# JacksonCampolattaro/spectrogram-rs

Hardware: AMD Instinct MI355X
Metric: STFT frames/sec (4096-pt, hop 256) (higher is better)
Workload: dtype f32

## Files before the change

bindings/rust/sgx_sys.rs:

```rust
use std::os::raw::{c_char, c_int, c_void};

#[repr(C)]
pub struct SgxConfig {
    pub struct_size: u32,
    pub sample_rate: f32, pub period: f32, pub stride: f32,
    pub window_samples: u32, pub hop_samples: u32, pub channels: u32, pub rows: u32,
    pub f_min: f64, pub f_max: f64,
    pub min_db: f32, pub max_db: f32,
    pub interp: u32, pub lut_index_mode: u32,
    pub device: i32, pub flags: u32,
}
#[repr(C)] pub struct SgxCtx { _private: [u8; 0] }
#[repr(C)] pub struct SgxFbank { _private: [u8; 0] }

extern "C" {
    pub fn sgx_config_init(cfg: *mut SgxConfig) -> c_int;
    pub fn sgx_create(cfg: *const SgxConfig, out: *mut *mut SgxCtx) -> c_int;
    pub fn sgx_destroy(ctx: *mut SgxCtx);
    pub fn sgx_last_error(ctx: *const SgxCtx) -> *const c_char;
    pub fn sgx_num_frames(ctx: *const SgxCtx, n_samples: usize) -> usize;
    pub fn sgx_process_one(ctx: *mut SgxCtx, h_lr: *const f32, n_avail: usize, h_out: *mut f32) -> c_int;
    pub fn sgx_stft_batch(ctx: *mut SgxCtx, d_pcm: *const f32, n_samples: usize, first_frame: usize,
                          max_frames: usize, d_mags: *mut f32, n_out: *mut usize) -> c_int;
    pub fn sgx_stft_batch_f16(ctx: *mut SgxCtx, d_pcm: *const f32, n_samples: usize, first_frame: usize,
                              max_frames: usize, d_mags_f16: *mut c_void, n_out: *mut usize) -> c_int;
    pub fn sgx_stft_batch_complex(ctx: *mut SgxCtx, d_pcm: *const f32, n_samples: usize, first_frame: usize,
                                  max_frames: usize, d_spec: *mut f32, n_out: *mut usize) -> c_int;
    pub fn sgx_istft_batch(ctx: *mut SgxCtx, d_spec: *const f32, n_frames: usize, first_sample: usize,
                           max_samples: usize, d_pcm: *mut f32, n_out: *mut usize) -> c_int;
    pub fn sgx_istft_supported(ctx: *const SgxCtx) -> c_int;
    pub fn sgx_render_batch(ctx: *mut SgxCtx, d_pcm: *const f32, n_samples: usize, first_frame: usize,
                            max_frames: usize, d_rgba: *mut u8, n_out: *mut usize) -> c_int;
    pub fn sgx_magnitude_in(ctx: *mut SgxCtx, d_mags: *const f32, n_columns: usize, h_ranges: *const f32,
                            n_ranges: u32, d_out: *mut f32) -> c_int;
    pub fn sgx_bands_batch(ctx: *mut SgxCtx, d_pcm: *const f32, n_samples: usize, first_frame: usize,
                           max_frames: usize, d_bands: *mut f32, n_out: *mut usize) -> c_int;
    pub fn sgx_bands_fused(ctx: *const SgxCtx) -> c_int;
    pub fn sgx_bands_peak_batch(ctx: *mut SgxCtx, d_pcm: *const f32, n_samples: usize, first_frame: usize, max_frames: usize,
                                group: usize, d_peak: *mut f32, n_out: *mut usize) -> c_int;
    pub fn sgx_bands_peak_fused(ctx: *const SgxCtx) -> c_int;
    pub fn sgx_psd_batch(ctx: *mut SgxCtx, d_pcm: *const f32, n_samples: usize, first_frame: usize, max_frames: usize,
                         group: usize, d_psd: *mut f32, n_out: *mut usize) -> c_int;
    pub fn sgx_csd_batch(ctx: *mut SgxCtx, d_pcm: *const f32, n_samples: usize, first_frame: usize, max_frames: usize,
                         group: usize, d_csd: *mut f32, n_out: *mut usize) -> c_int;
    pub fn sgx_psd_mags(ctx: *mut SgxCtx, d_mags: *const f32, n_frames: usize, group: usize, d_psd: *mut f32,
                        n_out: *mut usize) -> c_int;
    pub fn sgx_csd_spec(ctx: *mut SgxCtx, d_spec: *const f32, n_frames: usize, group: usize, d_csd: *mut f32,
                        n_out: *mut usize) -> c_int;
    pub fn sgx_psd_fused(ctx: *const SgxCtx) -> c_int;
    pub fn sgx_csd_fused(ctx: *const SgxCtx) -> c_int;
    pub fn sgx_render_bands(ctx: *mut SgxCtx, d_bands: *const f32, n_columns: usize, d_rgba: *mut u8) -> c_int;
    pub fn sgx_fbank_create(ctx: *mut SgxCtx, n_filters: u32, h_first: *const u32, h_count: *const u32, h_weights: *const f32,
                            power: u32, out_fbank: *mut *mut SgxFbank) -> c_int;
    pub fn sgx_fbank_destroy(fbank: *mut SgxFbank);
    pub fn sgx_fbank_filters(fbank: *const SgxFbank) -> u32;
    pub fn sgx_fbank_batch(fbank: *mut SgxFbank, d_pcm: *const f32, n_samples: usize, first_frame: usize, max_frames: usize,
                           d_out: *mut f32, n_out: *mut usize) -> c_int;
    pub fn sgx_fbank_mags(fbank: *mut SgxFbank, d_mags: *const f32, n_columns: usize, d_out: *mut f32) -> c_int;
    pub fn sgx_fbank_fused(fbank: *const SgxFbank) -> c_int;
    pub fn sgx_fbank_cross_batch(fbank: *mut SgxFbank, d_pcm: *const f32, n_samples: usize, first_frame: usize, max_frames: usize,
                                 d_out: *mut f32, n_out: *mut usize) -> c_int;
    pub fn sgx_fbank_cross_spec(fbank: *mut SgxFbank, d_spec: *const f32, n_columns: usize, d_out: *mut f32) -> c_int;
    pub fn sgx_fbank_cross_fused(fbank: *const SgxFbank) -> c_int;
    pub fn sgx_mel_weights(sample_rate: f64, window_samples: u32, n_mels: u32, f_min: f64, f_max: f64, scale: u32, norm: u32,
                           h_first: *mut u32, h_count: *mut u32, h_weights: *mut f32, n_weights: *mut usize) -> c_int;
    pub fn sgx_set_gradient(ctx: *mut SgxCtx, h_rgb: *const u8, n: u32, stereo: c_int) -> c_int;
    pub fn sgx_set_gradient_fn(ctx: *mut SgxCtx, eval: extern "C" fn(f64, *mut u8, *mut c_void), user: *mut c_void,
                               stereo: c_int) -> c_int;
    pub fn sgx_set_builtin_scheme(ctx: *mut SgxCtx, name: *const c_char, stereo: c_int) -> c_int;
    pub fn sgx_lookup_table(ctx: *mut SgxCtx, resolution: u32, h_out: *mut f32) -> c_int;
    pub fn sgx_sync(ctx: *mut SgxCtx) -> c_int;
    pub fn sgx_set_cu_limit(ctx: *mut SgxCtx, n: u32) -> c_int;
    pub fn sgx_cu_limit(ctx: *const SgxCtx) -> u32;
}
extern "C" {
    pub fn hipMalloc(p: *mut *mut c_void, bytes: usize) -> c_int;
    pub fn hipFree(p: *mut c_void) -> c_int;
    pub fn hipMemcpy(dst: *mut c_void, src: *const c_void, bytes: usize, kind: c_int) -> c_int;
}
pub const HIP_MEMCPY_HOST_TO_DEVICE: c_int = 1;
pub const HIP_MEMCPY_DEVICE_TO_HOST: c_int = 2;
pub const SGX_FLAG_PAIRED_FRAMES: u32 = 1024;
pub const SGX_FLAG_COMPLEX_MONO: u32 = 512;
pub const SGX_FLAG_LARGE_TRANSFORM: u32 = 4096;
pub const SGX_MEL_HTK: u32 = 0;
pub const SGX_MEL_SLANEY: u32 = 1;
pub const SGX_MEL_NORM_NONE: u32 = 0;
pub const SGX_MEL_NORM_SLANEY: u32 = 1;
pub const SGX_LIVE_BANDS: c_int = 3;
```

include/sgx.h:

```cpp
#ifndef SGX_H
#define SGX_H

#include <stddef.h>
#include <stdint.h>

#ifdef __cplusplus
extern "C" {
#endif

#if defined(__GNUC__)
#define SGX_API __attribute__((visibility("default")))
#else
#define SGX_API
#endif

typedef enum sgx_status {
    SGX_OK = 0,
    SGX_ERR_INVALID_ARG = -1,
    SGX_ERR_UNSUPPORTED = -2,
    SGX_ERR_HIP = -3,
    SGX_ERR_NOMEM = -4,
    SGX_ERR_NO_DEVICE = -5
} sgx_status;

#define SGX_INTERP_CUBIC 0u
#define SGX_INTERP_COSINE 1u

#define SGX_LUT_FLOOR_N 0u
#define SGX_LUT_ROUND_NM1 1u

typedef struct sgx_ctx sgx_ctx;

typedef struct sgx_config {
    uint32_t struct_size;
    float sample_rate;
    float period;
    float stride;
    uint32_t window_samples;
    uint32_t hop_samples;
    uint32_t channels;
    uint32_t rows;
    double f_min, f_max;
    float min_db, max_db;
    uint32_t interp;
    uint32_t lut_index_mode;
    int32_t device;
    uint32_t flags;
} sgx_config;

#define SGX_FLAG_FORCE_GENERIC 1u
#define SGX_FLAG_NO_FUSED_RENDER 4u
#define SGX_FLAG_PAIRED_FRAMES 1024u
#define SGX_FLAG_COMPLEX_MONO 512u
#define SGX_FLAG_LUT_WALK 64u
#define SGX_FLAG_MIXED_GENERIC 256u
#define SGX_FLAG_LARGE_TRANSFORM 4096u

typedef struct sgx_info {
    uint32_t struct_size;
    uint32_t window_samples;
    uint32_t fft_length;
    uint32_t num_frequencies;
    uint32_t hop_samples;
    uint32_t channels;
    uint32_t pairs;
    uint32_t rows;
    uint32_t sample_rate_u32;
    uint32_t total_samples_per_column;
    uint32_t stft_kernel;
    uint32_t render_path;
    uint64_t mags_bytes_per_frame;
    uint64_t rgba_bytes_per_frame;
} sgx_info;


SGX_API const char *sgx_version(void);

SGX_API int sgx_config_init(sgx_config *cfg);

SGX_API int sgx_create(const sgx_config *cfg, sgx_ctx **out_ctx);
SGX_API void sgx_destroy(sgx_ctx *ctx);

SGX_API const char *sgx_last_error(const sgx_ctx *ctx);

SGX_API int sgx_query(const sgx_ctx *ctx, sgx_info *out);

SGX_API size_t sgx_num_frames(const sgx_ctx *ctx, size_t n_samples);

SGX_API int sgx_set_stream(sgx_ctx *ctx, void *stream);
SGX_API int sgx_sync(sgx_ctx *ctx);

SGX_API int sgx_set_cu_limit(sgx_ctx *ctx, uint32_t n);
SGX_API uint32_t sgx_cu_limit(const sgx_ctx *ctx);


SGX_API int sgx_stft_batch(sgx_ctx *ctx, const float *d_pcm, size_t n_samples, size_t first_frame,
                           size_t max_frames, float *d_mags, size_t *n_out);

SGX_API int sgx_stft_batch_complex(sgx_ctx *ctx, const float *d_pcm, size_t n_samples, size_t first_frame,
                                   size_t max_frames, float *d_spec, size_t *n_out);

SGX_API int sgx_istft_batch(sgx_ctx *ctx, const float *d_spec, size_t n_frames, size_t first_sample,
                            size_t max_samples, float *d_pcm, size_t *n_out);
SGX_API int sgx_istft_supported(const sgx_ctx *ctx);

SGX_API int sgx_stft_batch_f16(sgx_ctx *ctx, const float *d_pcm, size_t n_samples, size_t first_frame,
                               size_t max_frames, void *d_mags_f16, size_t *n_out);

SGX_API int sgx_process_one(sgx_ctx *ctx, const float *h_lr, size_t n_avail, float *h_out);


SGX_API int sgx_render_batch(sgx_ctx *ctx, const float *d_pcm, size_t n_samples, size_t first_frame,
                             size_t max_frames, uint8_t *d_rgba, size_t *n_out);

SGX_API int sgx_render_mags(sgx_ctx *ctx, const float *d_mags, size_t n_columns, uint8_t *d_rgba);

SGX_API int sgx_magnitude_in(sgx_ctx *ctx, const float *d_mags, size_t n_columns, const float *h_ranges,
                             uint32_t n_ranges, float *d_out);

SGX_API int sgx_bands_batch(sgx_ctx *ctx, const float *d_pcm, size_t n_samples, size_t first_frame,
                            size_t max_frames, float *d_bands, size_t *n_out);
SGX_API int sgx_bands_fused(const sgx_ctx *ctx);

SGX_API int sgx_bands_peak_batch(sgx_ctx *ctx, const float *d_pcm, size_t n_samples, size_t first_frame, size_t max_frames,
                                 size_t group, float *d_peak, size_t *n_out);
SGX_API int sgx_bands_peak_fused(const sgx_ctx *ctx);

SGX_API int sgx_psd_batch(sgx_ctx *ctx, const float *d_pcm, size_t n_samples, size_t first_frame, size_t max_frames,
                          size_t group, float *d_psd, size_t *n_out);
SGX_API int sgx_csd_batch(sgx_ctx *ctx, const float *d_pcm, size_t n_samples, size_t first_frame, size_t max_frames,
                          size_t group, float *d_csd, size_t *n_out);
SGX_API int sgx_psd_mags(sgx_ctx *ctx, const float *d_mags, size_t n_frames, size_t group, float *d_psd, size_t *n_out);
SGX_API int sgx_csd_spec(sgx_ctx *ctx, const float *d_spec, size_t n_frames, size_t group, float *d_csd, size_t *n_out);
SGX_API int sgx_psd_fused(const sgx_ctx *ctx);
SGX_API int sgx_csd_fused(const sgx_ctx *ctx);
typedef struct sgx_fbank sgx_fbank;

SGX_API int sgx_fbank_create(sgx_ctx *ctx, uint32_t n_filters, const uint32_t *h_first, const uint32_t *h_count,
                             const float *h_weights, uint32_t power, void **out_fbank);
SGX_API void sgx_fbank_destroy(void *fbank);
SGX_API uint32_t sgx_fbank_filters(const void *fbank);
SGX_API int sgx_fbank_batch(void *fbank, const float *d_pcm, size_t n_samples, size_t first_frame, size_t max_frames,
                            float *d_out, size_t *n_out);
SGX_API int sgx_fbank_mags(void *fbank, const float *d_mags, size_t n_columns, float *d_out);
SGX_API int sgx_fbank_fused(const void *fbank);

SGX_API int sgx_fbank_cross_batch(void *fbank, const float *d_pcm, size_t n_samples, size_t first_frame, size_t max_frames,
                                  float *d_out, size_t *n_out);
SGX_API int sgx_fbank_cross_spec(void *fbank, const float *d_spec, size_t n_columns, float *d_out);
SGX_API int sgx_fbank_cross_fused(const void *fbank);

#define SGX_MEL_HTK 0u
#define SGX_MEL_SLANEY 1u
#define SGX_MEL_NORM_NONE 0u
#define SGX_MEL_NORM_SLANEY 1u
SGX_API int sgx_mel_weights(double sample_rate, uint32_t window_samples, uint32_t n_mels, double f_min, double f_max, uint32_t scale,
                            uint32_t norm, uint32_t *h_first, uint32_t *h_count, float *h_weights, size_t *n_weights);

SGX_API int sgx_render_bands(sgx_ctx *ctx, const float *d_bands, size_t n_columns, uint8_t *d_rgba);

SGX_API int sgx_spectrum_levels(sgx_ctx *ctx, const float *d_column, uint32_t n_bars, double *h_levels);


typedef struct sgx_live sgx_live;

#define SGX_LIVE_MAGS 0
#define SGX_LIVE_MAGS_F16 1
#define SGX_LIVE_RGBA 2
#define SGX_LIVE_BANDS 3

#define SGX_LIVE_REFERENCE_SKIP 1u

SGX_API int sgx_live_create(sgx_ctx *ctx, size_t capacity_pairs, uint32_t flags, sgx_live **out);
SGX_API void sgx_live_destroy(sgx_live *live);
SGX_API long long sgx_live_push(sgx_live *live, const float *h_samples, size_t n_values, uint32_t channels);
SGX_API size_t sgx_live_occupied(const sgx_live *live);
SGX_API int sgx_live_tick(sgx_live *live, int what, void *h_out, size_t max_frames, size_t *n_frames);


SGX_API int sgx_set_gradient(sgx_ctx *ctx, const uint8_t *h_rgb, uint32_t n, int stereo);
typedef void (*sgx_gradient_fn)(double t, uint8_t rgb_out[3], void *user);
SGX_API int sgx_set_gradient_fn(sgx_ctx *ctx, sgx_gradient_fn eval, void *user, int stereo);
SGX_API int sgx_set_builtin_gradient(sgx_ctx *ctx, const char *name);
SGX_API int sgx_set_builtin_scheme(sgx_ctx *ctx, const char *name, int stereo);
SGX_API int sgx_builtin_gradient_eval(const char *name, double t, uint8_t rgb_out[3]);
SGX_API int sgx_builtin_gradient(const char *name, uint8_t *h_rgb_out );

SGX_API int sgx_lookup_table(sgx_ctx *ctx, uint32_t resolution, float *h_out);


SGX_API int sgx_bin_edges(const sgx_ctx *ctx, float *h_out);
SGX_API int sgx_row_sample_counts(const sgx_ctx *ctx, uint32_t *h_out);
SGX_API int sgx_window(const sgx_ctx *ctx, float *h_out);

typedef struct sgx_view sgx_view;
SGX_API int sgx_view_create(sgx_ctx *ctx, uint32_t viewport_frames , sgx_view **out);
SGX_API void sgx_view_destroy(sgx_view *view);
SGX_API int sgx_view_write_rows(sgx_view *view, const void *d_rows_f16, size_t n_rows, uint32_t *offset_out);
SGX_API uint32_t sgx_view_offset(const sgx_view *view);
SGX_API int sgx_live_tick_view(sgx_live *live, sgx_view *view, size_t max_frames, size_t *n_frames);
SGX_API int sgx_view_draw(sgx_view *view, uint32_t width, uint32_t height, float *d_rgba_f32);

typedef struct sgx_image sgx_image;
SGX_API int sgx_image_create(sgx_ctx *ctx, uint32_t width , sgx_image **out);
SGX_API void sgx_image_destroy(sgx_image *image);
SGX_API int sgx_image_write_columns(sgx_image *image, const uint8_t *d_rgba, size_t n_columns, uint32_t *offset_out);
SGX_API uint32_t sgx_image_offset(const sgx_image *image);
SGX_API uint32_t sgx_image_width(const sgx_image *image);
SGX_API uint32_t sgx_image_height(const sgx_image *image);
SGX_API int sgx_live_tick_image(sgx_live *live, sgx_image *image, size_t max_frames, size_t *n_frames);
SGX_API int sgx_image_read(sgx_image *image, int scrolled, uint8_t *d_out);
SGX_API const uint8_t *sgx_image_pixels(const sgx_image *image);


SGX_API int sgx_synth_white_noise(sgx_ctx *ctx, float *d_out, uint64_t first, size_t n_samples,
                                  uint32_t channels, uint32_t seed);
SGX_API int sgx_checksum(sgx_ctx *ctx, const void *d_buf, size_t n_bytes, uint64_t base_word, uint64_t *h_out);
SGX_API int sgx_checksum_add(sgx_ctx *ctx, const void *d_buf, size_t n_bytes, uint64_t base_word, uint64_t *d_acc);

#ifdef __cplusplus
}
#endif
#endif
```

spectrogram_rs_amd/_lib.py:

```python
from __future__ import annotations

import ctypes as C
import os

_HERE = os.path.dirname(os.path.abspath(__file__))
LIB_PATH = os.environ.get("SGX_LIB", os.path.join(_HERE, "libsgx.so"))

SGX_OK = 0
SGX_ERR_INVALID_ARG = -1
SGX_ERR_UNSUPPORTED = -2
SGX_ERR_HIP = -3
SGX_ERR_NOMEM = -4
SGX_ERR_NO_DEVICE = -5

INTERP_CUBIC, INTERP_COSINE = 0, 1
LUT_FLOOR_N, LUT_ROUND_NM1 = 0, 1
FLAG_FORCE_GENERIC = 1
FLAG_NO_FUSED_RENDER = 4
FLAG_LUT_WALK = 64
FLAG_MIXED_GENERIC = 256
FLAG_COMPLEX_MONO = 512
FLAG_PAIRED_FRAMES = 1024
FLAG_LARGE_TRANSFORM = 4096
LIVE_MAGS, LIVE_MAGS_F16, LIVE_RGBA, LIVE_BANDS = 0, 1, 2, 3
LIVE_REFERENCE_SKIP = 1
MEL_HTK, MEL_SLANEY = 0, 1
MEL_NORM_NONE, MEL_NORM_SLANEY = 0, 1


class SgxError(RuntimeError):
    def __init__(self, code: int, message: str):
        super().__init__(f"sgx error {code}: {message}")
        self.code = code


class sgx_config(C.Structure):
    _fields_ = [
        ("struct_size", C.c_uint32),
        ("sample_rate", C.c_float),
        ("period", C.c_float),
        ("stride", C.c_float),
        ("window_samples", C.c_uint32),
        ("hop_samples", C.c_uint32),
        ("channels", C.c_uint32),
        ("rows", C.c_uint32),
        ("f_min", C.c_double),
        ("f_max", C.c_double),
        ("min_db", C.c_float),
        ("max_db", C.c_float),
        ("interp", C.c_uint32),
        ("lut_index_mode", C.c_uint32),
        ("device", C.c_int32),
        ("flags", C.c_uint32),
    ]


class sgx_info(C.Structure):
    _fields_ = [
        ("struct_size", C.c_uint32),
        ("window_samples", C.c_uint32),
        ("fft_length", C.c_uint32),
        ("num_frequencies", C.c_uint32),
        ("hop_samples", C.c_uint32),
        ("channels", C.c_uint32),
        ("pairs", C.c_uint32),
        ("rows", C.c_uint32),
        ("sample_rate_u32", C.c_uint32),
        ("total_samples_per_column", C.c_uint32),
        ("stft_kernel", C.c_uint32),
        ("render_path", C.c_uint32),
        ("mags_bytes_per_frame", C.c_uint64),
        ("rgba_bytes_per_frame", C.c_uint64),
    ]


_vp, _sz = C.c_void_p, C.c_size_t
_ctx = C.c_void_p
SIGNATURES = [
    ("sgx_version", C.c_char_p, []),
    ("sgx_config_init", C.c_int, [C.POINTER(sgx_config)]),
    ("sgx_create", C.c_int, [C.POINTER(sgx_config), C.POINTER(_ctx)]),
    ("sgx_destroy", None, [_ctx]),
    ("sgx_last_error", C.c_char_p, [_ctx]),
    ("sgx_query", C.c_int, [_ctx, C.POINTER(sgx_info)]),
    ("sgx_num_frames", _sz, [_ctx, _sz]),
    ("sgx_set_stream", C.c_int, [_ctx, _vp]),
    ("sgx_sync", C.c_int, [_ctx]),
    ("sgx_set_cu_limit", C.c_int, [_ctx, C.c_uint32]),
    ("sgx_cu_limit", C.c_uint32, [_ctx]),
    ("sgx_stft_batch", C.c_int, [_ctx, _vp, _sz, _sz, _sz, _vp, C.POINTER(_sz)]),
    ("sgx_stft_batch_f16", C.c_int, [_ctx, _vp, _sz, _sz, _sz, _vp, C.POINTER(_sz)]),
    ("sgx_stft_batch_complex", C.c_int, [_ctx, _vp, _sz, _sz, _sz, _vp, C.POINTER(_sz)]),
    ("sgx_istft_batch", C.c_int, [_ctx, _vp, _sz, _sz, _sz, _vp, C.POINTER(_sz)]),
    ("sgx_istft_supported", C.c_int, [_ctx]),
    ("sgx_process_one", C.c_int, [_ctx, _vp, _sz, _vp]),
    ("sgx_render_batch", C.c_int, [_ctx, _vp, _sz, _sz, _sz, _vp, C.POINTER(_sz)]),
    ("sgx_render_mags", C.c_int, [_ctx, _vp, _sz, _vp]),
    ("sgx_magnitude_in", C.c_int, [_ctx, _vp, _sz, _vp, C.c_uint32, _vp]),
    ("sgx_bands_batch", C.c_int, [_ctx, _vp, _sz, _sz, _sz, _vp, C.POINTER(_sz)]),
    ("sgx_bands_fused", C.c_int, [_ctx]),
    ("sgx_bands_peak_batch", C.c_int, [_ctx, _vp, _sz, _sz, _sz, _sz, _vp, C.POINTER(_sz)]),
    ("sgx_bands_peak_fused", C.c_int, [_ctx]),
    ("sgx_psd_batch", C.c_int, [_ctx, _vp, _sz, _sz, _sz, _sz, _vp, C.POINTER(_sz)]),
    ("sgx_csd_batch", C.c_int, [_ctx, _vp, _sz, _sz, _sz, _sz, _vp, C.POINTER(_sz)]),
    ("sgx_psd_mags", C.c_int, [_ctx, _vp, _sz, _sz, _vp, C.POINTER(_sz)]),
    ("sgx_csd_spec", C.c_int, [_ctx, _vp, _sz, _sz, _vp, C.POINTER(_sz)]),
    ("sgx_psd_fused", C.c_int, [_ctx]),
    ("sgx_csd_fused", C.c_int, [_ctx]),
    ("sgx_render_bands", C.c_int, [_ctx, _vp, _sz, _vp]),
    ("sgx_fbank_create", C.c_int, [_ctx, C.c_uint32, _vp, _vp, _vp, C.c_uint32, C.POINTER(_vp)]),
    ("sgx_fbank_destroy", None, [_vp]),
    ("sgx_fbank_filters", C.c_uint32, [_vp]),
    ("sgx_fbank_batch", C.c_int, [_vp, _vp, _sz, _sz, _sz, _vp, C.POINTER(_sz)]),
    ("sgx_fbank_mags", C.c_int, [_vp, _vp, _sz, _vp]),
    ("sgx_fbank_fused", C.c_int, [_vp]),
    ("sgx_fbank_cross_batch", C.c_int, [_vp, _vp, _sz, _sz, _sz, _vp, C.POINTER(_sz)]),
    ("sgx_fbank_cross_spec", C.c_int, [_vp, _vp, _sz, _vp]),
    ("sgx_fbank_cross_fused", C.c_int, [_vp]),
    ("sgx_mel_weights", C.c_int, [C.c_double, C.c_uint32, C.c_uint32, C.c_double, C.c_double, C.c_uint32, C.c_uint32, _vp, _vp, _vp,
                                  C.POINTER(_sz)]),
    ("sgx_spectrum_levels", C.c_int, [_ctx, _vp, C.c_uint32, _vp]),
    ("sgx_live_create", C.c_int, [_ctx, _sz, C.c_uint32, C.POINTER(_vp)]),
    ("sgx_live_destroy", None, [_vp]),
    ("sgx_live_push", C.c_longlong, [_vp, _vp, _sz, C.c_uint32]),
    ("sgx_live_occupied", _sz, [_vp]),
    ("sgx_live_tick", C.c_int, [_vp, C.c_int, _vp, _sz, C.POINTER(_sz)]),
    ("sgx_set_gradient", C.c_int, [_ctx, _vp, C.c_uint32, C.c_int]),
    ("sgx_set_gradient_fn", C.c_int, [_ctx, _vp, _vp, C.c_int]),
    ("sgx_set_builtin_gradient", C.c_int, [_ctx, C.c_char_p]),
    ("sgx_builtin_gradient", C.c_int, [C.c_char_p, _vp]),
    ("sgx_lookup_table", C.c_int, [_ctx, C.c_uint32, _vp]),
    ("sgx_bin_edges", C.c_int, [_ctx, _vp]),
    ("sgx_row_sample_counts", C.c_int, [_ctx, _vp]),
    ("sgx_window", C.c_int, [_ctx, _vp]),
    ("sgx_synth_white_noise", C.c_int, [_ctx, _vp, C.c_uint64, _sz, C.c_uint32, C.c_uint32]),
    ("sgx_set_builtin_scheme", C.c_int, [_ctx, C.c_char_p, C.c_int]),
    ("sgx_builtin_gradient_eval", C.c_int, [C.c_char_p, C.c_double, C.POINTER(C.c_uint8)]),
    ("sgx_view_create", C.c_int, [_ctx, C.c_uint32, C.POINTER(C.c_void_p)]),
    ("sgx_view_destroy", None, [C.c_void_p]),
    ("sgx_view_write_rows", C.c_int, [C.c_void_p, _vp, _sz, C.POINTER(C.c_uint32)]),
    ("sgx_view_offset", C.c_uint32, [C.c_void_p]),
    ("sgx_live_tick_view", C.c_int, [C.c_void_p, C.c_void_p, _sz, C.POINTER(_sz)]),
    ("sgx_view_draw", C.c_int, [C.c_void_p, C.c_uint32, C.c_uint32, _vp]),
    ("sgx_image_create", C.c_int, [_ctx, C.c_uint32, C.POINTER(C.c_void_p)]),
    ("sgx_image_destroy", None, [C.c_void_p]),
    ("sgx_image_write_columns", C.c_int, [C.c_void_p, _vp, _sz, C.POINTER(C.c_uint32)]),
    ("sgx_image_offset", C.c_uint32, [C.c_void_p]),
    ("sgx_image_width", C.c_uint32, [C.c_void_p]),
    ("sgx_image_height", C.c_uint32, [C.c_void_p]),
    ("sgx_live_tick_image", C.c_int, [C.c_void_p, C.c_void_p, _sz, C.POINTER(_sz)]),
    ("sgx_image_read", C.c_int, [C.c_void_p, C.c_int, _vp]),
    ("sgx_image_pixels", C.c_void_p, [C.c_void_p]),
    ("sgx_checksum", C.c_int, [_ctx, _vp, _sz, C.c_uint64, C.POINTER(C.c_uint64)]),
    ("sgx_checksum_add", C.c_int, [_ctx, _vp, _sz, C.c_uint64, _vp]),
]

GRADIENT_FN = C.CFUNCTYPE(None, C.c_double, C.POINTER(C.c_uint8), C.c_void_p)

_lib = None


def load():
    global _lib
    if _lib is not None:
        return _lib
    if not os.path.exists(LIB_PATH):
        raise ImportError(
            f"{LIB_PATH} is missing: build the HIP extension first "
            "(python -c 'import __graft_entry__ as g; g.build()' or make -C spectrogram_rs_amd/csrc). "
            "There is no CPU fallback."
        )
    import torch

    lib = C.CDLL(LIB_PATH, mode=C.RTLD_GLOBAL)
    for name, restype, argtypes in SIGNATURES:
        fn = getattr(lib, name)
        fn.restype = restype
        fn.argtypes = argtypes
    _lib = lib
    return lib
```

spectrogram_rs_amd/csrc/sgx_internal.hpp:

```cpp
#pragma once

#include <hip/hip_runtime.h>

#include <cstdint>
#include <array>
#include <memory>
#include <string>
#include <vector>

#include "../../include/sgx.h"
#include "device_buffer.hpp"
#include "unit_root.hpp"

namespace sgx {

#ifdef __HIPCC__
typedef float sgx_f2v __attribute__((ext_vector_type(2)));
__device__ __forceinline__ float2 cubic_pair(float2 y0, float2 y1, float2 y2, float2 y3, float mu, float mu2, float mu3)
{
    const sgx_f2v Y0 = {y0.x, y0.y}, Y1 = {y1.x, y1.y}, Y2 = {y2.x, y2.y}, Y3 = {y3.x, y3.y};
    const sgx_f2v a0 = ((Y3 - Y2) - Y0) + Y1;
    const sgx_f2v a1 = (Y0 - Y1) - a0;
    const sgx_f2v a2 = Y2 - Y0;
    const sgx_f2v r = ((a0 * mu3) + (a1 * mu2)) + ((a2 * mu) + Y1);
    return make_float2(r.x, r.y);
}
#endif

constexpr int kTCells = 512;
__host__ __device__ inline int sgx_t_cell(double t)
{
    const double x = (t + 1.0) * (double)(kTCells / 2);
    return x >= (double)kTCells ? kTCells - 1 : (x > 0.0 ? (int)x : 0);
}

struct RowEntry {
    uint32_t first;
    uint32_t count;
    float count_f;
    uint32_t pad;
};

struct SampleEntry {
    int32_t i0;
    union { int32_t i1; float w0; };
    float w1;
    float w2;
};
static_assert(sizeof(SampleEntry) == 16, "SampleEntry must be 16 bytes");

struct Tables {
    std::vector<float> window;
    std::vector<float2> twiddle;
    std::vector<float> edges;
    std::vector<RowEntry> rows;
    std::vector<SampleEntry> samples;
};

struct Palette {
    std::vector<uint8_t> rgb;
    uint32_t n = 0;
    int stereo = 0;
    std::vector<float> lut_thr;
    std::vector<float> alpha_thr;
    bool segments = false;
    sgx_gradient_fn fn = nullptr;
    void *fn_user = nullptr;
    std::vector<double> t_thr;
    std::vector<uint16_t> t_cell;
    uint8_t nan_rgb[3] = {0, 0, 0};
};

void build_tables(uint32_t W, uint32_t R, uint32_t sample_rate_u32, double f_min, double f_max, uint32_t interp,
                  Tables &out);
void build_range_tables(uint32_t W, uint32_t sample_rate_u32, uint32_t interp, const float *range_f0, const float *range_f1,
                        uint32_t n_ranges, std::vector<RowEntry> &rows, std::vector<SampleEntry> &samples);
void build_palette_thresholds(float min_db, float max_db, uint32_t lut_mode, Palette &pal);
void build_palette_segments(float min_db, float max_db, Palette &pal);
int lut_index_host(double t, uint32_t n, uint32_t mode);
uint8_t alpha_u8_host(float alpha);
float bounded_db_host(float min_db, float max_db, float power);

enum StftKernel : int { kKernelGeneric = 0, kKernelWg4096 = 2, kKernelChirp = 4, kKernelMixed = 6, kKernelW4800 = 9, kKernelW16384 = 10, kKernelLarge = 11 };

namespace wg { struct WgTables; }
namespace wgr { struct RealTables; }
namespace mix { struct MixTables; struct ChirpTables; }
namespace w48 { struct W48Tables; }
namespace blu { struct BluTables; }
namespace w16k { struct TablesW; }
namespace large { struct LargeTables; }
namespace istft { struct ITables; }
struct TablesDelete {
    void operator()(wg::WgTables *t) const;
    void operator()(wgr::RealTables *t) const;
    void operator()(mix::MixTables *t) const;
    void operator()(mix::ChirpTables *t) const;
    void operator()(w48::W48Tables *t) const;
    void operator()(blu::BluTables *t) const;
    void operator()(w16k::TablesW *t) const;
    void operator()(large::LargeTables *t) const;
    void operator()(istft::ITables *t) const;
};
template <typename T> using TablesPtr = std::unique_ptr<T, TablesDelete>;

inline float2 unit_root2(unsigned long long e, unsigned long long n) { const UnitRoot w = unit_root(e, n); return make_float2(w.re, w.im); }

}

struct sgx_ctx {
    sgx_config cfg{};
    uint32_t W = 0, P = 0, M = 0, H = 0, C = 0, pairs = 0, R = 0, sr_u32 = 0, logP = 0;
    int device = 0;
    hipStream_t stream = nullptr;
    hipEvent_t rebind_event = nullptr;
    sgx::StftKernel stft_kernel = sgx::kKernelGeneric;

    sgx::Tables tab;
    sgx::Palette pal;

    sgx::DeviceBuffer<float> d_window;
    sgx::DeviceBuffer<float2> d_twiddle;
    sgx::DeviceBuffer<sgx::RowEntry> d_rows;
    sgx::DeviceBuffer<sgx::SampleEntry> d_samples;
    sgx::DeviceBuffer<float> d_lut_thr;
    sgx::DeviceBuffer<float> d_alpha_thr;
    sgx::DeviceBuffer<uchar4> d_lut_rgba;
    sgx::DeviceBuffer<uint2> d_pal_seed;
    sgx::DeviceBuffer<double> d_t_thr;
    sgx::DeviceBuffer<uint16_t> d_t_cell;
    sgx::TablesPtr<sgx::wg::WgTables> wg;
    sgx::TablesPtr<sgx::blu::BluTables> blu;
    sgx::TablesPtr<sgx::mix::MixTables> mix;
    sgx::TablesPtr<sgx::w48::W48Tables> w4800;
    sgx::TablesPtr<sgx::wgr::RealTables> real;
    sgx::TablesPtr<sgx::mix::ChirpTables> chz;
    sgx::TablesPtr<sgx::w16k::TablesW> w16k;
    sgx::TablesPtr<sgx::large::LargeTables> large;
    sgx::TablesPtr<sgx::istft::ITables> istft;

    sgx::DeviceBuffer<float> d_ws_mags;
    sgx::DeviceBuffer<float> d_one_in, d_one_out;
    sgx::DeviceBuffer<unsigned long long> d_cksum;
    std::vector<float> bands_key;
    sgx::DeviceBuffer<sgx::RowEntry> d_band_rows;
    sgx::DeviceBuffer<sgx::SampleEntry> d_band_samples;
    sgx::DeviceBuffer<float> d_levels;
    sgx::DeviceBuffer<double> d_psd_carry;

    unsigned long long palette_gen = 0;

    int n_cu = 256;
    int n_cu_device = 256;
    size_t lds_optin = 64 * 1024;
    mutable std::vector<std::pair<std::array<size_t, 3>, int>> occupancy_cache;
    std::vector<struct sgx_view *> views;
    std::vector<struct sgx_image *> images;
    std::vector<struct sgx_fbank *> fbanks;

    std::string err;

    ~sgx_ctx();
};

namespace sgx {

enum class Out { kMags, kMagsF16, kComplex, kRgba, kBands, kPeak, kFbank, kFbankCross, kPsd, kCsd };
struct StftCall {
    const float *pcm;
    uint32_t channels, pairs;
    size_t first, n, total;
    void *out;
    Out kind;
    size_t peak_group;
    const struct sgx_fbank *bank = nullptr;
};
hipError_t launch_generic(const sgx_ctx *c, const StftCall &call);
hipError_t launch_wg4096(const sgx_ctx *c, const StftCall &call);
hipError_t launch_w16384(const sgx_ctx *c, const StftCall &call);
hipError_t launch_w4800(const sgx_ctx *c, const StftCall &call);
hipError_t launch_mixed(const sgx_ctx *c, const StftCall &call);
hipError_t launch_chirpz(const sgx_ctx *c, const StftCall &call);
hipError_t launch_bluestein(const sgx_ctx *c, const StftCall &call);
hipError_t launch_large(const sgx_ctx *c, const StftCall &call);

inline bool paired_mono(const sgx_ctx *c, uint32_t channels)
{
    return channels == 1 && (c->cfg.flags & SGX_FLAG_PAIRED_FRAMES) && !(c->cfg.flags & SGX_FLAG_COMPLEX_MONO);
}
inline bool descriptor_pairs_fit(uint32_t H, uint32_t W) { return 4ull * ((unsigned long long)H + W) <= 0x7fffffffull; }
struct RunSplit { unsigned long long per, blocks; };
inline RunSplit runs_of(unsigned long long n_jobs, unsigned long long per) { return {per, (n_jobs + per - 1) / per}; }
inline RunSplit run_split(const sgx_ctx *c, unsigned long long n_jobs, unsigned per_cu)
{
    const unsigned long long blocks = (unsigned long long)c->n_cu * per_cu, per = (n_jobs + blocks - 1) / blocks;
    return runs_of(n_jobs, per < 1 ? 1 : per);
}
inline bool fast4096_supported(const sgx_ctx *c) { return c->W == 2048; }
hipError_t wg4096_init(sgx_ctx *c);
bool wg4096_can_fuse_render(const sgx_ctx *c);
bool wg4096_can_fuse_bands(const sgx_ctx *c);
bool wg4096_can_fuse_peak(const sgx_ctx *c);
hipError_t launch_deinterleave_pairs(const sgx_ctx *c, const float *d_pcm, float *d_planes, size_t plane_floats, size_t first_sample, size_t n_samples,
                                     uint32_t channels, uint32_t pairs);
bool wg4096_seed_is_within_one(const sgx_ctx *c);
void lut_seed_coefficients(const sgx_ctx *c, float &a, float &b);
namespace wg { bool seed_within_one(const std::vector<float> &thr, double guess_a, double guess_b); }
bool w16384_supported(const sgx_ctx *c);
hipError_t w16384_init(sgx_ctx *c);
hipError_t real4096_init(sgx_ctx *c);
bool real4096_serves(const sgx_ctx *c, const float *d_pcm, uint32_t channels);
bool w4800_supported(const sgx_ctx *c);
hipError_t w4800_init(sgx_ctx *c);
bool mixed_supported(uint32_t W);
hipError_t mixed_init(sgx_ctx *c);
hipError_t mixed_length_tables(uint32_t n, TablesPtr<mix::MixTables> &out);
uint32_t mixed_fixed_plan(const sgx_ctx *c);
bool mixed_real_serves(const sgx_ctx *c, uint32_t channels);
bool chirpz_supported(uint32_t W);
hipError_t chirpz_init(sgx_ctx *c);
bool chirpz_real_serves(const sgx_ctx *c, uint32_t channels);
bool mixed_can_fuse_render(const sgx_ctx *c);
bool mixed_can_fuse_bands(const sgx_ctx *c);
bool bluestein_supported(uint32_t W);
hipError_t bluestein_init(sgx_ctx *c);
bool large_supported(uint32_t W);
hipError_t large_init(sgx_ctx *c);
int istft_route(const sgx_ctx *c);
hipError_t istft_init(sgx_ctx *c);
hipError_t launch_istft(const sgx_ctx *c, const float *d_spec, size_t n_frames, size_t s0, size_t s1, float *d_pcm);
hipError_t launch_to_half(const sgx_ctx *c, const float *d_in, void *d_out, size_t n_pairs);
hipError_t launch_render(const sgx_ctx *c, const float *d_mags, size_t n_columns, uint8_t *d_rgba);
hipError_t launch_magnitude_in(const sgx_ctx *c, const float *d_mags, size_t n_columns, const RowEntry *d_rows,
                               const SampleEntry *d_samples, uint32_t n_ranges, float *d_out);
inline size_t peak_columns(size_t n_src, size_t group, size_t sub)
{
    const size_t spc = (group + sub - 1) / sub, full = n_src / group, rem = n_src - full * group;
    return full * spc + (rem + sub - 1) / sub;
}
hipError_t launch_bands_peak(const sgx_ctx *c, const float *d_src, size_t n_src, size_t group, size_t sub, float *d_dst, bool accumulate);
hipError_t launch_render_bands(const sgx_ctx *c, const float *d_bands, size_t n_columns, uint8_t *d_rgba);
void detach_views(sgx_ctx *c);
void detach_images(sgx_ctx *c);
sgx_ctx *image_context(const struct sgx_image *im);
sgx_ctx *view_context(const struct sgx_view *v);
hipError_t launch_white_noise(const sgx_ctx *c, float *d_out, uint64_t first, size_t n, uint32_t channels, uint32_t seed);
hipError_t launch_checksum(const sgx_ctx *c, const uint32_t *d_words, size_t n_words, uint64_t base_word,
                           unsigned long long *d_acc);

}

#ifdef __HIPCC__
__device__ __forceinline__ void st_stream(float2 *p, float a, float b)
{
    *p = make_float2(a, b);
}

#if SGX_STAMPS
#define SGX_STAMP(i) { const unsigned long long now_ = __builtin_readcyclecounter(); st_acc[i] += now_ - st_last; st_last = now_; }
#else
#define SGX_STAMP(i)
#endif
#endif
```

spectrogram_rs_amd/csrc/stft4096_real.hip:

```cpp
#include <cmath>
#include <type_traits>

#include "stft4096_wg.hpp"

namespace sgx {

namespace wgr {

using wg::kBufComplex;
using wg::kLdsBytes;
using wg::kLdsBytesRender;
using wg::kM;
using wg::kS1;
using wg::kS2;
using wg::kW;
using wg::lds_barrier;
using wg::lds_read_alone;
using wg::lds_cfloat2;
using wg::lds_ptr;
using wg::pcm_rsrc;
using wg::u32x2;
using wg::u32x4;

typedef float f2v __attribute__((ext_vector_type(2)));
__device__ __forceinline__ float cl_fma(float a, float c, float u) { return fmaf(a, c, u); }
__device__ __forceinline__ f2v cl_fma(f2v a, float c, f2v u) { return __builtin_elementwise_fma(a, f2v{c, c}, u); }

#include "fft_codelets.inc"

using wg::Params;

__device__ __forceinline__ float2 cmulf(float2 a, float2 b)
{
    return make_float2(fmaf(a.x, b.x, -(a.y * b.y)), fmaf(a.x, b.y, a.y * b.x));
}

__device__ __forceinline__ __amdgpu_buffer_rsrc_t out_rsrc(char *base, long long byte, bool present)
{
    const uint32_t lo = __builtin_amdgcn_readfirstlane((uint32_t)byte);
    const uint32_t hi = __builtin_amdgcn_readfirstlane((uint32_t)((unsigned long long)byte >> 32));
    const int records = __builtin_amdgcn_readfirstlane(present ? 0x7fffffff : 0);
    return __builtin_amdgcn_make_buffer_rsrc(base + (long long)(((unsigned long long)hi << 32) | lo), 0, records, 0x00020000);
}

__device__ __forceinline__ void fft8_half_zero(const float (&zr)[4], const float (&zi)[4], float (&yr)[8], float (&yi)[8])
{
    constexpr float kH = 0.70710678118654752440f;
    auto fft4 = [](float a0r, float a0i, float a1r, float a1i, float a2r, float a2i, float a3r, float a3i, float *outr, float *outi) {
        const float s0r = a0r + a2r, s0i = a0i + a2i, s1r = a0r - a2r, s1i = a0i - a2i;
        const float s2r = a1r + a3r, s2i = a1i + a3i, s3r = a1r - a3r, s3i = a1i - a3i;
        outr[0] = s0r + s2r; outi[0] = s0i + s2i;
        outr[4] = s0r - s2r; outi[4] = s0i - s2i;
        outr[2] = s1r + s3i; outi[2] = s1i - s3r;
        outr[6] = s1r - s3i; outi[6] = s1i + s3r;
    };
    fft4(zr[0], zi[0], zr[1], zi[1], zr[2], zi[2], zr[3], zi[3], yr, yi);
    const float y1r = (zr[1] + zi[1]) * kH, y1i = (zi[1] - zr[1]) * kH;
    const float y3r = (zi[3] - zr[3]) * kH, y3i = -(zr[3] + zi[3]) * kH;
    fft4(zr[0], zi[0], y1r, y1i, zi[2], -zr[2], y3r, y3i, yr + 1, yi + 1);
}

constexpr int kRowsF32 = 0, kRowsF16 = 1, kPixels = 2;
constexpr int kBands = 3;
constexpr int kPeak = 5;
constexpr int kFbank = 6;
constexpr int kRowsC64 = 4;

constexpr int kPlaneIm = 4480;
constexpr int kBufComplexTR = kPlaneIm;
static_assert(kBufComplexTR >= kBufComplex && 16 * 280 <= kPlaneIm, "the planes hold both images");
constexpr size_t kLdsBytesR = (size_t)(kBufComplexTR + 256) * sizeof(float2);
constexpr size_t kLdsBytesRenderR = kLdsBytesR + 256 * sizeof(uint2);
static_assert(4 * kLdsBytesRenderR <= 160 * 1024, "four workgroups per CU");
template <int STRIDE>
__device__ __forceinline__ void addtid_rows(float2 a, float2 b, uint32_t m0_wave, int ra, int rb)
{
    asm volatile("s_mov_b32 m0, %4\n\t"
                 "s_nop 0\n\t"
                 "ds_write_addtid_b32 %0 offset:%5\n\t"
                 "ds_write_addtid_b32 %1 offset:%6\n\t"
                 "ds_write_addtid_b32 %2 offset:%7\n\t"
                 "ds_write_addtid_b32 %3 offset:%8"
                 :
                 : "v"(a.x), "v"(a.y), "v"(b.x), "v"(b.y), "s"(m0_wave), "i"(4 * STRIDE * ra), "i"(4 * STRIDE * ra + 4 * kPlaneIm), "i"(4 * STRIDE * rb), "i"(4 * STRIDE * rb + 4 * kPlaneIm)
                 : "memory");
}
__device__ __forceinline__ void read_planes(const float4 *rd4, float (&xr)[16], float (&xi)[16])
{
#pragma unroll
    for (int c = 0; c < 4; ++c) {
        const float4 r = rd4[c], i = rd4[c + kPlaneIm / 4];
        xr[4 * c] = r.x; xr[4 * c + 1] = r.y; xr[4 * c + 2] = r.z; xr[4 * c + 3] = r.w;
        xi[4 * c] = i.x; xi[4 * c + 1] = i.y; xi[4 * c + 2] = i.z; xi[4 * c + 3] = i.w;
    }
}
__device__ __forceinline__ float lane_xor8(float v) { return __int_as_float(__builtin_amdgcn_mov_dpp(__float_as_int(v), 0x128, 0xf, 0xf, true)); }

#if SGX_STAMPS
__device__ unsigned long long g_phase_cycles_r[24];
#endif

template <int MODE, int PIX, bool SLIDE>
__global__ void __launch_bounds__(256, 4) stft4096_real_kernel(Params p)
{
    extern __shared__ __attribute__((aligned(16))) unsigned char smem_raw[];
    float2 *buf = reinterpret_cast<float2 *>(smem_raw);
    constexpr bool TR = SLIDE;
    float2 *tw2 = buf + (TR ? kBufComplexTR : kBufComplex);
    uint2 *pal = reinterpret_cast<uint2 *>(tw2 + 256);
    constexpr bool F16 = MODE == kRowsF16;
    constexpr bool C64 = MODE == kRowsC64;
    constexpr bool FUSED = MODE == kPixels || MODE == kBands || MODE == kPeak || MODE == kFbank;

    const int tid = threadIdx.x;
    const int t_p1 = TR ? (tid >> 4) + 16 * (tid & 15) : tid;
    float *plane = reinterpret_cast<float *>(smem_raw);
    const uint32_t m0_wave = __builtin_amdgcn_readfirstlane((uint32_t)(tid >> 6) * 272u);
    const float4 *rd4_1 = reinterpret_cast<const float4 *>(plane + 272 * (tid >> 4) + 68 * ((tid & 15) >> 2) + 16 * (tid & 3));
    const float4 *rd4_2 = reinterpret_cast<const float4 *>(plane + 280 * ((tid & 127) >> 3) + 68 * ((8 * (tid >> 7) + (tid & 7)) >> 2) + 16 * (tid & 3));
    tw2[tid] = p.tw2[tid];
    uint32_t row_words[4] = {0u, 0u, 0u, 0u};
    if (FUSED && MODE != kFbank) {
        if (MODE == kPixels) pal[tid] = make_uint2(__float_as_uint(tid < 255 ? p.lut_thr[tid] : __builtin_nanf("")), *reinterpret_cast<const uint32_t *>(&p.lut_rgba[tid]));
#pragma unroll
        for (int i = 0; i < 4; ++i)
            if ((uint32_t)tid + 256u * i < p.R) row_words[i] = p.rows[tid + 256 * i];
    }

    float win[8];
#pragma unroll
    for (int a = 0; a < 4; ++a) {
        win[2 * a] = p.window[2 * t_p1 + 512 * a] * (1.0f / 2048.0f);
        win[2 * a + 1] = p.window[2 * t_p1 + 512 * a + 1] * (1.0f / 2048.0f);
    }
    float2 tw1[8];
#pragma unroll
    for (int q = 1; q < 8; ++q) tw1[q] = p.tw1[q * 256 + t_p1];
    const int F = tid >> 7, u = tid & 127;
    float2 twu[8];
#pragma unroll
    for (int q = 0; q < 8; ++q) twu[q] = p.twu[q * 128 + u];
    const int g2 = tid >> 4, t0_2 = tid & 15;
    const int cbase2 = (g2 >> 3) * 128 + (g2 & 7);
    __syncthreads();

    const unsigned long long job_begin = (unsigned long long)blockIdx.x * p.jobs_per_block;
    unsigned long long job_end = job_begin + p.jobs_per_block;
    if (job_end > p.n_jobs) job_end = p.n_jobs;
#ifdef SGX_VARIANT_SKIP_LAST_JOB
    if (job_end > job_begin + 1) --job_end;
#endif
    if (job_begin >= job_end) return;

    auto samples_from = [&](unsigned long long first) {
        const unsigned long long left = first < p.stream_samples ? (p.stream_samples - first) * 4 : 0;
        const unsigned long long addr = (unsigned long long)(p.pcm + (first < p.stream_samples ? first : 0));
        const uint32_t lo = __builtin_amdgcn_readfirstlane((uint32_t)addr), hi = __builtin_amdgcn_readfirstlane((uint32_t)(addr >> 32));
        const int records = __builtin_amdgcn_readfirstlane((int)(left < 0x7fffffffull ? left : 0x7fffffffull));
        return __builtin_amdgcn_make_buffer_rsrc(reinterpret_cast<void *>(((unsigned long long)hi << 32) | lo), 0, records, 0x00020000);
    };
    auto columns_from = [&](unsigned long long col0) { return samples_from(2 * col0); };
    auto column = [&](__amdgpu_buffer_rsrc_t r, int byte_offset) {
        const u32x2 v = __builtin_amdgcn_raw_buffer_load_b64(r, t_p1 * 8, byte_offset, 0);
        return make_float2(__uint_as_float(v.x), __uint_as_float(v.y));
    };
    float2 R[8];
    float2 L;
    auto load_pair = [&](unsigned long long fa_) {
        const __amdgpu_buffer_rsrc_t r0 = samples_from(fa_ * p.H), r1 = samples_from((fa_ + 1) * p.H);
#pragma unroll
        for (int a = 0; a < 4; ++a) { R[2 * a] = column(r0, 2048 * a); R[2 * a + 1] = column(r1, 2048 * a); }
    };
    {
        const __amdgpu_buffer_rsrc_t r0 = columns_from(128 * (p.first_frame + 2 * job_begin));
        if (SLIDE) {
#pragma unroll
            for (int j = 0; j < 8; ++j) R[j] = column(r0, 1024 * j);
            L = column(r0, 9216);
        } else {
            load_pair(p.first_frame + 2 * job_begin);
            L = R[7];
        }
#pragma unroll
        for (int j = 0; j < 8; ++j) asm volatile("" ::"v"(R[j].x), "v"(R[j].y));
        asm volatile("" ::"v"(L.x), "v"(L.y));
#pragma unroll
        for (int q = 1; q < 8; ++q) asm volatile("" ::"v"(tw1[q].x), "v"(tw1[q].y));
#pragma unroll
        for (int q = 0; q < 8; ++q) asm volatile("" ::"v"(twu[q].x), "v"(twu[q].y), "v"(win[q]));
    }
    float2 *xch = buf + 2304;

    char *out = reinterpret_cast<char *>(p.mags);
    constexpr int kBin = C64 ? 16 : (F16 ? 4 : 8);
#if SGX_STAMPS
    unsigned long long st_acc[20] = {0, 0, 0, 0, 0, 0, 0, 0, 0, 0, 0, 0, 0, 0, 0, 0, 0, 0, 0, 0};
    unsigned long long st_last = __builtin_readcyclecounter();
#endif
    for (unsigned long long job = job_begin; job < job_end; ++job) {
        SGX_STAMP(19)
        const unsigned long long fa = p.first_frame + 2 * job;
        const unsigned long long la = 2 * job, lb = la + 1;
        const bool have_b = lb < p.n_frames;

        float yr[8], yi[8];
        {
            float zr[4], zi[4];
#pragma unroll
            for (int a = 0; a < 4; ++a) { zr[a] = R[2 * a].x * win[2 * a]; zi[a] = R[2 * a].y * win[2 * a + 1]; }
            fft8_half_zero(zr, zi, yr, yi);
        }
        float vr[8], vi[8];
        {
            float zr[4], zi[4];
#pragma unroll
            for (int a = 0; a < 4; ++a) { zr[a] = R[2 * a + 1].x * win[2 * a]; zi[a] = R[2 * a + 1].y * win[2 * a + 1]; }
            fft8_half_zero(zr, zi, vr, vi);
        }
        SGX_STAMP(0)
        lds_barrier();
        SGX_STAMP(1)
#pragma unroll
        for (int q = 0; q < 8; ++q) {
            const float2 ya = make_float2(yr[q], yi[q]), yb = make_float2(vr[q], vi[q]);
            if (TR) {
                addtid_rows<272>(q == 0 ? ya : cmulf(ya, tw1[q]), q == 0 ? yb : cmulf(yb, tw1[q]), m0_wave, q, 8 + q);
            } else {
                buf[q * kS1 + tid] = q == 0 ? ya : cmulf(ya, tw1[q]);
                buf[(8 + q) * kS1 + tid] = q == 0 ? yb : cmulf(yb, tw1[q]);
            }
        }
        __builtin_amdgcn_s_setprio(0);
        SGX_STAMP(2)
        lds_barrier();
        SGX_STAMP(3)

        float xr[16], xi[16];
        if (TR) {
            read_planes(rd4_1, xr, xi);
        } else {
#pragma unroll
            for (int t1 = 0; t1 < 16; ++t1) {
                const float2 v = buf[g2 * kS1 + t0_2 + 16 * t1];
                xr[t1] = v.x; xi[t1] = v.y;
            }
        }
        fft16(xr, xi);
        SGX_STAMP(4)
        lds_barrier();
        SGX_STAMP(5)
        if (TR) {
            lds_cfloat2 *tw2p = lds_ptr(tw2 + t0_2);
#pragma unroll
            for (int q2 = 0; q2 < 16; q2 += 2) {
                const int pa = FFT16_OUT[q2], pb = FFT16_OUT[q2 + 1];
                const float2 va = make_float2(xr[pa], xi[pa]), vb = make_float2(xr[pb], xi[pb]);
                addtid_rows<280>(q2 == 0 ? va : cmulf(va, lds_read_alone(tw2p, q2 * 16)), cmulf(vb, lds_read_alone(tw2p, (q2 + 1) * 16)), m0_wave, q2, q2 + 1);
            }
        } else {
#pragma unroll
            for (int q2 = 0; q2 < 16; ++q2) {
                const int pos = FFT16_OUT[q2];
                const float2 v = make_float2(xr[pos], xi[pos]);
                buf[t0_2 * kS2 + cbase2 + 8 * q2] = q2 == 0 ? v : cmulf(v, tw2[q2 * 16 + t0_2]);
            }
        }
        SGX_STAMP(6)
        lds_barrier();
        SGX_STAMP(7)

        if (TR) {
            read_planes(rd4_2, xr, xi);
        } else {
#pragma unroll
            for (int t0 = 0; t0 < 16; ++t0) {
                const float2 v = buf[t0 * kS2 + tid];
                xr[t0] = v.x; xi[t0] = v.y;
            }
        }
        fft16(xr, xi);

        float2 Ln = make_float2(0.0f, 0.0f);
        if (SLIDE && !FUSED) Ln = column(columns_from(128 * (fa + 2) + 1152), 0);
        if (!SLIDE) load_pair(fa + 2);

        if (FUSED) __builtin_amdgcn_s_setprio(1);
        else __builtin_amdgcn_s_setprio(3);
        SGX_STAMP(8)
        lds_barrier();
        SGX_STAMP(9)
#pragma unroll
        for (int j = 0; j < 8; ++j) {
            const int pos = FFT16_OUT[8 + j];
            buf[j * 256 + tid] = make_float2(xr[pos], xi[pos]);
        }
        if (SLIDE && !TR) {
            xch[tid].x = tid < 128 ? L.x : R[7].x;
            xch[tid].y = tid < 128 ? L.y : R[7].y;
        }
        SGX_STAMP(10)
        lds_barrier();
        SGX_STAMP(11)
        if (SLIDE) {
            const float2 Y = TR ? make_float2(lane_xor8((tid & 8) ? R[7].x : L.x), lane_xor8((tid & 8) ? R[7].y : L.y)) : xch[(tid + 128) & 255];
#pragma unroll
            for (int j = 0; j < 6; ++j) R[j] = R[j + 2];
            R[6] = Y;
            R[7] = L;
        }

        const int pcol = F * 128 + (u == 0 ? 256 : 128 - u);
        float m1[8], m2[8];
        constexpr bool kInterleave = (!FUSED && SLIDE) || C64;
        const long long row = (long long)(F == 0 ? la : lb) * (long long)kM * kBin - kBin;
        const __amdgpu_buffer_rsrc_t r = out_rsrc(out, !FUSED ? row : 0, !FUSED && (F == 0 || have_b));
        const int l1 = kBin * u, l2 = kBin * (1152 - u);
        auto store_pair = [&](const int q3) {
            const float a = m1[q3], b = (q3 == 0 && u == 0) ? m1[0] : m2[q3];
            const int o1 = (q3 == 0 && u == 0) ? kBin * 1024 : l1;
            const int o2 = (q3 == 0 && u == 0) ? kBin * 128 : l2;
            const int s1 = kBin * 128 * q3, s2 = kBin * 128 * (7 - q3);
            if (F16) {
                const __half2 ha = __floats2half2_rn(a, a), hb = __floats2half2_rn(b, b);
                __builtin_amdgcn_raw_buffer_store_b32(*reinterpret_cast<const uint32_t *>(&ha), r, o1 + (s1 & 2047), s1 & ~2047, 0);
                __builtin_amdgcn_raw_buffer_store_b32(*reinterpret_cast<const uint32_t *>(&hb), r, o2 + (s2 & 2047), s2 & ~2047, 0);
            } else {
                __builtin_amdgcn_raw_buffer_store_b64(u32x2{__float_as_uint(a), __float_as_uint(a)}, r, o1 + (s1 & 2047), s1 & ~2047, 0);
                __builtin_amdgcn_raw_buffer_store_b64(u32x2{__float_as_uint(b), __float_as_uint(b)}, r, o2 + (s2 & 2047), s2 & ~2047, 0);
            }
        };
        float2 pvs[8];
        if (kInterleave) {
#pragma unroll
            for (int q3 = 0; q3 < 8; ++q3) pvs[q3] = buf[(7 - q3) * 256 + pcol];
        }
#pragma unroll
        for (int q3 = 0; q3 < 8; ++q3) {
            const int pos = FFT16_OUT[q3];
            float zr_ = xr[pos], zi_ = xi[pos];
            float2 pv = kInterleave ? pvs[q3] : buf[(7 - q3) * 256 + pcol];
            if (q3 == 0) {
                const float2 own = buf[F * 128];
                const int p8 = FFT16_OUT[8];
                zr_ = u == 0 ? xr[p8] : zr_; zi_ = u == 0 ? xi[p8] : zi_;
                pv.x = u == 0 ? own.x : pv.x; pv.y = u == 0 ? own.y : pv.y;
            }
            const float er = zr_ + pv.x, ei = zi_ - pv.y;
            const float orr = zi_ + pv.y, oi = pv.x - zr_;
            const float wr = fmaf(twu[q3].x, orr, -(twu[q3].y * oi)), wi = fmaf(twu[q3].x, oi, twu[q3].y * orr);
            const float ar = er + wr, ai = ei + wi, br = er - wr, bi = ei - wi;
            if constexpr (C64) {
                const bool self = q3 == 0 && u == 0;
                const float cr2 = self ? ar : br, ci2 = self ? ai : -bi;
                const int o1 = self ? kBin * 1024 : l1, o2 = self ? kBin * 128 : l2;
                const int s1 = kBin * 128 * q3, s2 = kBin * 128 * (7 - q3);
                __builtin_amdgcn_raw_buffer_store_b128(u32x4{__float_as_uint(ar), __float_as_uint(ai), __float_as_uint(ar), __float_as_uint(ai)}, r, o1 + s1, 0, 0);
                __builtin_amdgcn_raw_buffer_store_b128(u32x4{__float_as_uint(cr2), __float_as_uint(ci2), __float_as_uint(cr2), __float_as_uint(ci2)}, r, o2 + s2, 0, 0);
                __builtin_amdgcn_sched_barrier(0);
                continue;
            }
            m1[q3] = __builtin_amdgcn_sqrtf(fmaf(ar, ar, ai * ai));
            m2[q3] = __builtin_amdgcn_sqrtf(fmaf(br, br, bi * bi));
            if (kInterleave) {
                store_pair(q3);
                __builtin_amdgcn_sched_barrier(0);
            }
        }

        if (!FUSED) {
            if (!kInterleave) {
#pragma unroll
                for (int q3 = 0; q3 < 8; ++q3) store_pair(q3);
            }
        } else {
            float2 *mpair = buf;
            float2 *vbuf = mpair + wg::kColSlots;
            float *mcol = reinterpret_cast<float *>(buf) + F;
            lds_barrier();
            SGX_STAMP(13)
            constexpr bool kEarlyWords = PIX != wg::kPixGeneric && MODE != kFbank;
            wg::SampleWords sw;
            const __amdgpu_buffer_rsrc_t rt_words = wg::pcm_rsrc(reinterpret_cast<const float *>(p.samples));
            int tid_w = tid;
            asm volatile("" : "+v"(tid_w));
#pragma unroll
            for (int q3 = 0; q3 < 8; ++q3) {
                const bool self = q3 == 0 && u == 0;
                const int k1 = self ? 1024 : u + 128 * q3, k2 = self ? 1024 : 2048 - u - 128 * q3;
                mcol[2 * k1] = m1[q3];
                mcol[2 * k2] = self ? m1[0] : m2[q3];
                if (q3 == 0 && u == 1) {
                    mcol[0] = m1[0];
                    mcol[2 * (kM + 1)] = mcol[2 * (kM + 2)] = m2[0];
                }
                if (kEarlyWords) {
                    sw.se[q3] = wg::sample_word(rt_words, p, (uint32_t)tid_w + 256u * q3);
                    __builtin_amdgcn_sched_barrier(0);
                }
            }
            if (kEarlyWords) sw.se[8] = wg::sample_word(rt_words, p, (uint32_t)tid_w + 2048u);
            static_assert(wg::kSampleSteps == 9 && wg::kSampleEarly == 9, "one word per column-write step and one behind them");
            SGX_STAMP(14)
            lds_barrier();
            SGX_STAMP(15)
            if constexpr (MODE == kFbank) {
                float2 *sums = reinterpret_cast<float2 *>(p.rgba);
                __builtin_amdgcn_s_setprio(3);
                fbank::filter_pass<true>(mpair + 1, reinterpret_cast<const fbank::Filter *>(p.rows), reinterpret_cast<const float *>(p.samples), p.R,
                                         p.interp == 2u, sums + la * (size_t)p.R, sums + lb * (size_t)p.R, true, have_b, (uint32_t)tid, 4u);
                if (SLIDE) L = column(columns_from(128 * (fa + 2) + 1152), 0);
            } else {
            if (kEarlyWords) wg::sample_pass_with<PIX>(p, mpair, vbuf, tid, sw);
            else wg::sample_pass<PIX>(p, mpair, vbuf, tid);
            [[maybe_unused]] wg::PeakDst peak_a{}, peak_b{};
            [[maybe_unused]] wg::PeakOld<true> peak_old{};
            if constexpr (MODE == kPeak) {
                peak_a = wg::peak_dst(p, la);
                peak_b = have_b ? wg::peak_dst_next(p, peak_a, lb) : peak_a;
                peak_old = wg::peak_prefetch<true>(p, peak_a, tid);
            }
            if (SLIDE) L = column(columns_from(128 * (fa + 2) + 1152), 0);
            SGX_STAMP(16)
            lds_barrier();
            SGX_STAMP(17)
            __builtin_amdgcn_s_setprio(3);
            if constexpr (MODE == kPeak) {
                wg::row_pass_peak<true>(p, row_words, vbuf, peak_a, peak_b, peak_old, have_b, tid);
            } else if constexpr (MODE == kBands) {
                float2 *bands = reinterpret_cast<float2 *>(p.rgba);
                wg::row_pass_bands<true>(p, row_words, vbuf, bands + la * (size_t)p.R, bands + lb * (size_t)p.R, true, have_b, tid);
            } else {
                uchar4 *rgba = reinterpret_cast<uchar4 *>(p.rgba);
                wg::row_pass<true, PIX>(p, row_words, vbuf, rgba + la * (size_t)p.R, rgba + lb * (size_t)p.R, true, have_b, pal, tid);
            }
            }
        }
        if (SLIDE && !FUSED) {
            asm volatile("" : "+v"(Ln.x), "+v"(Ln.y));
            L = Ln;
        }
        SGX_STAMP(18)
    }
#if SGX_STAMPS
    if ((tid & 63) == 0) {
#pragma unroll
        for (int i = 0; i < 20; ++i) atomicAdd(&g_phase_cycles_r[i], st_acc[i]);
        atomicAdd(&g_phase_cycles_r[20], (unsigned long long)(job_end - job_begin));
    }
#endif
}

struct RealTables {
    DeviceBuffer<float2> d_tw1, d_tw2, d_twu;
};

}

#if SGX_STAMPS
extern "C" __attribute__((visibility("default"))) int sgx_debug_phase_cycles_r(unsigned long long *h_out, int reset)
{
    hipError_t e = hipMemcpyFromSymbol(h_out, HIP_SYMBOL(wgr::g_phase_cycles_r), sizeof(unsigned long long) * 24);
    if (e == hipSuccess && reset) {
        unsigned long long zero[24] = {0};
        e = hipMemcpyToSymbol(HIP_SYMBOL(wgr::g_phase_cycles_r), zero, sizeof(zero));
    }
    return e == hipSuccess ? 0 : -1;
}
#endif

void TablesDelete::operator()(wgr::RealTables *t) const { delete t; }

hipError_t real4096_init(sgx_ctx *c)
{
    using namespace wgr;
    TablesPtr<RealTables> t(new RealTables());
    std::vector<float2> tw1(8 * 256), tw2(256), twu(8 * 128);
    for (int q = 0; q < 8; ++q)
        for (int tt = 0; tt < 256; ++tt) tw1[q * 256 + tt] = unit_root2((unsigned long long)tt * q, 2048);
    for (int q = 0; q < 16; ++q)
        for (int t0 = 0; t0 < 16; ++t0) tw2[q * 16 + t0] = unit_root2((unsigned long long)t0 * q, 256);
    for (int q3 = 0; q3 < 8; ++q3)
        for (int uu = 0; uu < 128; ++uu) twu[q3 * 128 + uu] = unit_root2((unsigned long long)(uu + 128 * q3), 4096);
    twu[0] = unit_root2(1024, 4096);
    hipError_t e = t->d_tw1.upload(tw1);
    if (e == hipSuccess) e = t->d_tw2.upload(tw2);
    if (e == hipSuccess) e = t->d_twu.upload(twu);
    if (e == hipSuccess) c->real = std::move(t);
    return e;
}

bool real4096_serves(const sgx_ctx *c, const float *d_pcm, uint32_t channels)
{
    (void)d_pcm;
    return channels == 1 && c->real && c->W == (uint32_t)wgr::kW;
}

namespace wg {

hipError_t launch_real4096(const sgx_ctx *c, Params p, Out kind)
{
    using namespace wgr;
    if (p.n_frames == 0) return hipSuccess;
    const RealTables *t = c->real.get();
    const bool hold_peak = kind == Out::kPeak;
    p.tw1 = t->d_tw1.get();
    p.tw2 = t->d_tw2.get();
    p.twu = t->d_twu.get();
    p.stream_samples = p.total_frames ? (p.total_frames - 1) * (unsigned long long)c->H + (unsigned long long)kW : 0;
    p.n_jobs = (p.n_frames + 1) / 2;
    RunSplit runs = run_split(c, p.n_jobs, 4);
    if (hold_peak) {
        runs = runs_of(p.n_jobs, peak_align_run(runs.per, 2, p.peak_group));
        p.peak_run = 2 * runs.per;
    }
    p.jobs_per_block = runs.per;
    const dim3 grid((unsigned)runs.blocks), block(256);
    auto launch = [&](auto slide_c) {
        constexpr bool S_ = decltype(slide_c)::value;
        constexpr size_t lds_rows = S_ ? kLdsBytesR : kLdsBytes, lds_render = S_ ? kLdsBytesRenderR : kLdsBytesRender;
        if (hold_peak) {
            if (p.interp == SGX_INTERP_COSINE) hipLaunchKernelGGL((stft4096_real_kernel<kPeak, kPixPeakCosine, S_>), grid, block, lds_rows, c->stream, p);
            else hipLaunchKernelGGL((stft4096_real_kernel<kPeak, kPixPeakCubic, S_>), grid, block, lds_rows, c->stream, p);
        } else if (kind == Out::kFbank) {
            hipLaunchKernelGGL((stft4096_real_kernel<kFbank, kPixFbank, S_>), grid, block, lds_rows, c->stream, p);
        } else if (kind == Out::kBands) {
            if (p.interp == SGX_INTERP_COSINE) hipLaunchKernelGGL((stft4096_real_kernel<kBands, kPixBandsCosine, S_>), grid, block, lds_rows, c->stream, p);
            else hipLaunchKernelGGL((stft4096_real_kernel<kBands, kPixBandsCubic, S_>), grid, block, lds_rows, c->stream, p);
        } else if (kind == Out::kRgba) {
            if (!p.seed_pm1) hipLaunchKernelGGL((stft4096_real_kernel<kPixels, kPixGeneric, S_>), grid, block, lds_render, c->stream, p);
            else if (p.interp == SGX_INTERP_COSINE) hipLaunchKernelGGL((stft4096_real_kernel<kPixels, kPixCosine, S_>), grid, block, lds_render, c->stream, p);
            else hipLaunchKernelGGL((stft4096_real_kernel<kPixels, kPixCubic, S_>), grid, block, lds_render, c->stream, p);
        } else if (kind == Out::kComplex) {
            hipLaunchKernelGGL((stft4096_real_kernel<kRowsC64, kPixNone, S_>), grid, block, lds_rows, c->stream, p);
        } else if (kind == Out::kMagsF16) {
            hipLaunchKernelGGL((stft4096_real_kernel<kRowsF16, kPixNone, S_>), grid, block, lds_rows, c->stream, p);
        } else {
            hipLaunchKernelGGL((stft4096_real_kernel<kRowsF32, kPixNone, S_>), grid, block, lds_rows, c->stream, p);
        }
    };
    if (c->H == 256) launch(std::true_type{});
    else launch(std::false_type{});
    const hipError_t e = hipGetLastError();
    return e == hipSuccess && hold_peak ? launch_peak_combine(c, p, runs.blocks) : e;
}

}

}
```

spectrogram_rs_amd/csrc/stft4096_wg.hpp:

```cpp
#pragma once
#include <hip/hip_fp16.h>

#include "sgx_fbank.hpp"
#include "sgx_internal.hpp"

namespace sgx {
namespace wg {

constexpr int kW = 2048, kP = 4096, kM = 2047;
constexpr bool kSlideWindow = true;
constexpr int kS1 = 272;
constexpr int kS2 = 257;
constexpr int kBufComplex = 16 * kS1;
constexpr size_t kLdsBytes = (size_t)(kBufComplex + 256) * sizeof(float2);
constexpr size_t kLdsBytesRender = kLdsBytes + 256 * sizeof(uint2);

struct PackedSample {
    int32_t i0;
    float w;
};

struct Params {
    const float *pcm;
    const float2 *tw1;
    const float2 *tw2;
    const float *window;
    union {
        float *mags;
        float2 *peak_partial;
    };
    unsigned long long first_frame, n_frames, n_jobs, jobs_per_block;
    unsigned long long pair_base;
    unsigned long long total_frames;
    uint32_t H, C, pair_l, pair_r, pairs, pair;
    uint32_t out_f16;
    const uint32_t *rows;
    const PackedSample *samples;
    uint32_t n_samples;
    union {
        const float *lut_thr;
        unsigned long long peak_group;
    };
    union {
        const uchar4 *lut_rgba;
        unsigned long long peak_run;
    };
    uint8_t *rgba;
    uint32_t R, interp;
    float guess_a, guess_b;
    uint32_t seed_pm1;
    uint32_t single_rows;
    uint32_t block_max_cnt;
    const float2 *twu;
    unsigned long long stream_samples;
};
static_assert(sizeof(Params) == 216, "the kernel argument of every instantiation: its size is part of their code objects");

inline unsigned long long peak_align_run(unsigned long long per, unsigned fpj, unsigned long long group)
{
    const unsigned long long unit = group % fpj == 0 ? group : group * fpj, run = per * fpj;
    if (unit > run / 32) return per;
    return (run + unit - 1) / unit * unit / fpj;
}
hipError_t launch_peak_combine(const sgx_ctx *c, const Params &p, unsigned long long blocks);

hipError_t launch_real4096(const sgx_ctx *c, Params p, Out kind);

constexpr int kPairAdjacentRow = 0, kPairAdjacent = 1;

struct WgTables {
    DeviceBuffer<float2> d_tw1, d_tw2;
    DeviceBuffer<uint32_t> d_rows;
    DeviceBuffer<PackedSample> d_samples;
    uint32_t n_samples = 0;
    uint32_t single_rows = 0;
    uint32_t block_max_cnt = 0;
    bool fusable = false;
    DeviceBuffer<float> d_planes;
    DeviceBuffer<float2> d_peak_partial;
};

__device__ __forceinline__ void lds_barrier()
{
    asm volatile("s_waitcnt lgkmcnt(0)\n\ts_barrier" ::: "memory");
}

typedef float lds_f2v __attribute__((ext_vector_type(2)));
typedef const lds_f2v __attribute__((address_space(3))) lds_cfloat2;
__device__ __forceinline__ lds_cfloat2 *lds_ptr(const float2 *p) { return (lds_cfloat2 *)p; }
__device__ __forceinline__ float2 lds_read_alone(lds_cfloat2 *&base, int idx)
{
    asm("" : "+v"(base));
    const lds_f2v v = base[idx];
    return make_float2(v.x, v.y);
}

typedef unsigned int u32x2 __attribute__((ext_vector_type(2)));
typedef unsigned int u32x4 __attribute__((ext_vector_type(4)));

__device__ __forceinline__ __amdgpu_buffer_rsrc_t row_rsrc(char *mags, long long row_byte, bool present = true)
{
    const uint32_t olo = __builtin_amdgcn_readfirstlane((uint32_t)row_byte);
    const uint32_t ohi = __builtin_amdgcn_readfirstlane((uint32_t)((unsigned long long)row_byte >> 32));
    const int records = __builtin_amdgcn_readfirstlane(present ? 0x7fffffff : 0);
    return __builtin_amdgcn_make_buffer_rsrc(mags + (long long)(((unsigned long long)ohi << 32) | olo), 0, records, 0x00020000);
}

__device__ __forceinline__ __amdgpu_buffer_rsrc_t pcm_rsrc(const float *base)
{
    const unsigned long long a = (unsigned long long)base;
    const uint32_t lo = __builtin_amdgcn_readfirstlane((uint32_t)a), hi = __builtin_amdgcn_readfirstlane((uint32_t)(a >> 32));
    return __builtin_amdgcn_make_buffer_rsrc(reinterpret_cast<void *>(((unsigned long long)hi << 32) | lo), 0, 0x7fffffff, 0x00020000);
}

constexpr int kAuxNt = 2;
template <bool DUP>
__device__ __forceinline__ void store_row(char *mags, long long row_byte, int col, const float (&va)[8], const float (&vb)[8], bool present = true)
{
    const __amdgpu_buffer_rsrc_t r = row_rsrc(mags, row_byte, present);
    const int lane_off = col * 8;
    const int lane_off0 = col != 0 ? lane_off : (int)0x80000000;
#pragma unroll
    for (int q3 = 0; q3 < 8; ++q3) {
        const u32x2 d = {__float_as_uint(va[q3]), __float_as_uint(DUP ? va[q3] : vb[q3])};
        __builtin_amdgcn_raw_buffer_store_b64(d, r, (q3 == 0 ? lane_off0 : lane_off) + 2048 * (q3 & 1), 4096 * (q3 >> 1), DUP ? 0 : kAuxNt);
    }
}

constexpr int kColSlots = 2050;
constexpr int kMaxFusedSamples = kBufComplex - kColSlots;
constexpr int kPixNone = 0, kPixCubic = 1, kPixCosine = 2, kPixGeneric = 3, kPixRowsF16 = 4;
constexpr int kPixBandsCubic = 5, kPixBandsCosine = 6;
constexpr int kPixPeakCubic = 8, kPixPeakCosine = 9;
constexpr bool pix_peak(int pix) { return pix == kPixPeakCubic || pix == kPixPeakCosine; }
constexpr bool pix_bands(int pix) { return pix == kPixBandsCubic || pix == kPixBandsCosine || pix_peak(pix); }
constexpr bool pix_cosine(int pix) { return pix == kPixCosine || pix == kPixBandsCosine || pix == kPixPeakCosine; }
constexpr int kPixFbank = 10;
constexpr int kPixFbankCross = 11;
static_assert(2 * kColSlots <= kBufComplex, "the two product columns lie in the transform's buffer");
constexpr int kPixRowsC64 = 7;


template <bool COSINE>
__device__ __forceinline__ float2 interp_sample2(const float2 *P, int i0, float w)
{
    float2 v;
    if (COSINE) {
        const float w1 = 1.0f - w;
        lds_cfloat2 *q = lds_ptr(P + i0);
        const float2 a = lds_read_alone(q, 1), b = lds_read_alone(q, 2);
        v.x = a.x * w1 + b.x * w;
        v.y = a.y * w1 + b.y * w;
    } else {
        const float mu = w, mu2 = mu * mu, mu3 = mu * mu2;
        lds_cfloat2 *q = lds_ptr(P + i0);
        asm("" : "+v"(q)); const lds_f2v y0 = q[0];
        asm("" : "+v"(q)); const lds_f2v y1 = q[1];
        asm("" : "+v"(q)); const lds_f2v y2 = q[2];
        asm("" : "+v"(q)); const lds_f2v y3 = q[3];
        const lds_f2v a0 = ((y3 - y2) - y0) + y1;
        const lds_f2v a1 = (y0 - y1) - a0;
        const lds_f2v a2 = y2 - y0;
        const lds_f2v r = ((a0 * mu3) + (a1 * mu2)) + ((a2 * mu) + y1);
        v.x = r.x; v.y = r.y;
    }
    return v;
}

template <bool COSINE>
__device__ __forceinline__ void sample_pass_for(const Params &p, const float2 *P, float2 *vbuf, int tid)
{
    const __amdgpu_buffer_rsrc_t rt = pcm_rsrc(reinterpret_cast<const float *>(p.samples));
    auto item = [&](uint32_t i) {
        const u32x2 v = __builtin_amdgcn_raw_buffer_load_b64(rt, (int)((i < p.n_samples ? i : 0u) * 8u), 0, 0);
        return PackedSample{(int32_t)v.x, __uint_as_float(v.y)};
    };
    constexpr int kSteps = (kMaxFusedSamples + 255) / 256, kAhead = 9;
    PackedSample se[kSteps];
    asm volatile("" : "+v"(tid));
#pragma unroll
    for (int k = 0; k < kAhead && k < kSteps; ++k) se[k] = item(tid + 256 * k);
#pragma unroll
    for (int k = 0; k < kSteps; ++k) {
        if (k + kAhead < kSteps) se[k + kAhead] = item(tid + 256 * (k + kAhead));
        const uint32_t s = tid + 256 * k;
        if (s < p.n_samples) vbuf[s] = interp_sample2<COSINE>(P, se[k].i0, se[k].w);
        __builtin_amdgcn_sched_barrier(0);
    }
}

constexpr int kSampleSteps = (kMaxFusedSamples + 255) / 256;
constexpr int kSampleEarly = 9;
struct SampleWords { PackedSample se[kSampleEarly]; };
__device__ __forceinline__ PackedSample sample_word(const __amdgpu_buffer_rsrc_t &rt, const Params &p, uint32_t i)
{
    const u32x2 v = __builtin_amdgcn_raw_buffer_load_b64(rt, (int)((i < p.n_samples ? i : 0u) * 8u), 0, 0);
    return PackedSample{(int32_t)v.x, __uint_as_float(v.y)};
}
__device__ __forceinline__ void sample_request(const Params &p, int tid, SampleWords &w)
{
    const __amdgpu_buffer_rsrc_t rt = pcm_rsrc(reinterpret_cast<const float *>(p.samples));
    asm volatile("" : "+v"(tid));
#pragma unroll
    for (int k = 0; k < kSampleEarly; ++k) w.se[k] = sample_word(rt, p, tid + 256 * k);
}
template <int PIX>
__device__ __forceinline__ void sample_pass_with(const Params &p, const float2 *P, float2 *vbuf, int tid, const SampleWords &w)
{
    const __amdgpu_buffer_rsrc_t rt = pcm_rsrc(reinterpret_cast<const float *>(p.samples));
    asm volatile("" : "+v"(tid));
    PackedSample se[kSampleSteps];
#pragma unroll
    for (int k = 0; k < kSampleSteps; ++k) se[k] = k < kSampleEarly ? w.se[k] : sample_word(rt, p, tid + 256 * k);
#pragma unroll
    for (int k = 0; k < kSampleSteps; ++k) {
        const uint32_t s = tid + 256 * k;
        if (s < p.n_samples) {
            if (pix_cosine(PIX) || (PIX == kPixGeneric && p.interp == SGX_INTERP_COSINE)) vbuf[s] = interp_sample2<true>(P, se[k].i0, se[k].w);
            else vbuf[s] = interp_sample2<false>(P, se[k].i0, se[k].w);
        }
        __builtin_amdgcn_sched_barrier(0);
    }
}

template <int PIX>
__device__ __forceinline__ void sample_pass(const Params &p, const float2 *P, float2 *vbuf, int tid)
{
    if (pix_cosine(PIX) || (PIX == kPixGeneric && p.interp == SGX_INTERP_COSINE)) sample_pass_for<true>(p, P, vbuf, tid);
    else sample_pass_for<false>(p, P, vbuf, tid);
}

template <int PIX>
__device__ __forceinline__ uint32_t pixel_from_power(const Params &p, float power, const uint2 *pal)
{
    const float u = fmaf(__builtin_amdgcn_logf(power + 1e-7f), p.guess_a, p.guess_b);
    if (PIX != kPixGeneric || p.seed_pm1) {
        int idx = (int)floorf(u - 0.5f);
        idx = idx < 0 ? 0 : (idx > 254 ? 254 : idx);
        const uint2 e0 = pal[idx], e1 = pal[idx + 1];
        return power >= __uint_as_float(e0.x) ? e1.y : e0.y;
    }
    int idx = (int)floorf(u);
    idx = idx < 0 ? 0 : (idx > 255 ? 255 : idx);
    while (idx < 255 && power >= __uint_as_float(pal[idx].x)) ++idx;
    while (idx > 0 && !(power >= __uint_as_float(pal[idx - 1].x))) --idx;
    return pal[idx].y;
}

template <int PIX>
__device__ __forceinline__ uint32_t pixel_for(const Params &p, float l, float r, const uint2 *pal)
{
    return pixel_from_power<PIX>(p, (l * l) + (r * r), pal);
}

bool seed_within_one(const std::vector<float> &lut_thr, double guess_a, double guess_b);

template <bool MONO, int PIX>
__device__ __forceinline__ void row_pass(const Params &p, const uint32_t (&row_words)[4], const float2 *vbuf, uchar4 *dst_a, uchar4 *dst_b,
                                         bool have_a, bool have_b, const uint2 *pal, int tid)
{
    uint32_t *out_a = reinterpret_cast<uint32_t *>(dst_a), *out_b = reinterpret_cast<uint32_t *>(dst_b);
#pragma unroll 1
    for (int i_row = 0; i_row < 4; ++i_row) {
        const uint32_t py = tid + 256 * i_row;
        if (py >= p.R) break;
        const uint32_t re = i_row == 0 ? row_words[0] : i_row == 1 ? row_words[1] : i_row == 2 ? row_words[2] : row_words[3];
        const uint32_t first = re & 0xffffu, cnt = re >> 16;
        float l, r;
        if (p.single_rows & (1u << i_row)) {
            const float2 v = vbuf[first];
            l = v.x;
            r = v.y;
        } else {
            float sl = 0.0f, sr = 0.0f;
            for (uint32_t i = 0; i < cnt; ++i) {
                const float2 v = vbuf[first + i];
                sl = sl + v.x;
                sr = sr + v.y;
            }
            l = sl;
            r = sr;
            if (cnt > 1) {
                const float nf = (float)cnt;
                l = sl / nf;
                r = sr / nf;
            }
        }
        const uint32_t y = p.R - 1 - py;
        if (MONO) {
            if (have_a) out_a[y] = pixel_for<PIX>(p, l, l, pal);
            if (have_b) out_b[y] = pixel_for<PIX>(p, r, r, pal);
        } else {
            out_a[y] = pixel_for<PIX>(p, l, r, pal);
        }
        asm volatile("" ::: "memory");
    }
}

template <bool MONO>
__device__ __forceinline__ void row_pass_bands(const Params &p, const uint32_t (&row_words)[4], const float2 *vbuf, float2 *dst_a, float2 *dst_b,
                                               bool have_a, bool have_b, int tid)
{
#pragma unroll 1
    for (int i_row = 0; i_row < 4; ++i_row) {
        const uint32_t py = tid + 256 * i_row;
        if (py >= p.R) break;
        const uint32_t re = i_row == 0 ? row_words[0] : i_row == 1 ? row_words[1] : i_row == 2 ? row_words[2] : row_words[3];
        const uint32_t first = re & 0xffffu, cnt = re >> 16;
        float l, r;
        if (p.single_rows & (1u << i_row)) {
            const float2 v = vbuf[first];
            l = 0.0f + v.x;
            r = 0.0f + v.y;
        } else {
            float sl = 0.0f, sr = 0.0f;
            for (uint32_t i = 0; i < cnt; ++i) {
                const float2 v = vbuf[first + i];
                sl = sl + v.x;
                sr = sr + v.y;
            }
            l = sl;
            r = sr;
            if (cnt > 1) {
                const float nf = (float)cnt;
                l = sl / nf;
                r = sr / nf;
            }
        }
        if (MONO) {
            if (have_a) dst_a[py] = make_float2(l, l);
            if (have_b) dst_b[py] = make_float2(r, r);
        } else {
            dst_a[py] = make_float2(l, r);
        }
        asm volatile("" ::: "memory");
    }
}

struct PeakDst {
    float2 *col;
    bool first;
    unsigned long long end;
};
__device__ __forceinline__ PeakDst peak_dst(const Params &p, unsigned long long f)
{
    const unsigned long long run0 = (unsigned long long)blockIdx.x * p.peak_run;
    unsigned long long run1 = run0 + p.peak_run;
    if (run1 > p.n_frames) run1 = p.n_frames;
    const unsigned long long j = ((f | p.peak_group) >> 32) == 0 ? (unsigned long long)((uint32_t)f / (uint32_t)p.peak_group) : f / p.peak_group;
    const unsigned long long c0 = j * p.peak_group;
    unsigned long long c1 = c0 + p.peak_group;
    if (c1 > p.n_frames) c1 = p.n_frames;
    PeakDst d;
    if (c0 >= run0 && c1 <= run1) d.col = reinterpret_cast<float2 *>(p.rgba) + (j * p.pairs + p.pair) * (size_t)p.R;
    else d.col = p.peak_partial + ((size_t)blockIdx.x * 2 + (c0 >= run0 ? 1 : 0)) * (size_t)p.R;
    d.first = f == (c0 > run0 ? c0 : run0);
    d.end = c1;
    return d;
}
__device__ __forceinline__ PeakDst peak_dst_next(const Params &p, const PeakDst &a, unsigned long long f)
{
    if (f >= a.end) return peak_dst(p, f);
    PeakDst d = a;
    d.first = false;
    return d;
}

template <bool MONO>
struct PeakOld {
    float x0, x1, x2, x3, y0, y1, y2, y3;
};
template <bool MONO>
__device__ __forceinline__ void peak_prefetch_row(const Params &p, const PeakDst &d, uint32_t py, float &x, float &y)
{
    x = y = 0.0f;
    if (!d.first && py < p.R) {
        if (MONO) {
            x = reinterpret_cast<const float *>(d.col + py)[0];
        } else {
            const float2 v = d.col[py];
            x = v.x;
            y = v.y;
        }
    }
}
template <bool MONO>
__device__ __forceinline__ PeakOld<MONO> peak_prefetch(const Params &p, const PeakDst &d, int tid)
{
    PeakOld<MONO> o;
    asm volatile("" : "+v"(tid));
    peak_prefetch_row<MONO>(p, d, tid, o.x0, o.y0);
    peak_prefetch_row<MONO>(p, d, tid + 256, o.x1, o.y1);
    peak_prefetch_row<MONO>(p, d, tid + 512, o.x2, o.y2);
    peak_prefetch_row<MONO>(p, d, tid + 768, o.x3, o.y3);
    return o;
}

__device__ __forceinline__ void peak_update(float2 *col, uint32_t py, bool first, float l, float r)
{
    if (!first) {
        const float2 old = col[py];
        l = l > old.x ? l : old.x;
        r = r > old.y ? r : old.y;
    }
    col[py] = make_float2(l, r);
}

template <bool MONO>
__device__ __forceinline__ void row_pass_peak(const Params &p, const uint32_t (&row_words)[4], const float2 *vbuf, PeakDst a, PeakDst b,
                                              const PeakOld<MONO> &old, bool have_b, int tid)
{
    const bool same = MONO && have_b && a.col == b.col;
    float ox = old.x0, ox1 = old.x1, ox2 = old.x2, ox3 = old.x3;
    [[maybe_unused]] float oy = old.y0, oy1 = old.y1, oy2 = old.y2, oy3 = old.y3;
#pragma unroll 1
    for (int i_row = 0; i_row < 4; ++i_row) {
        const uint32_t py = tid + 256 * i_row;
        if (py >= p.R) break;
        const uint32_t re = i_row == 0 ? row_words[0] : i_row == 1 ? row_words[1] : i_row == 2 ? row_words[2] : row_words[3];
        const uint32_t first = re & 0xffffu, cnt = re >> 16;
        float l, r;
        if (p.single_rows & (1u << i_row)) {
            const float2 v = vbuf[first];
            l = 0.0f + v.x;
            r = 0.0f + v.y;
        } else {
            float sl = 0.0f, sr = 0.0f;
            for (uint32_t i = 0; i < cnt; ++i) {
                const float2 v = vbuf[first + i];
                sl = sl + v.x;
                sr = sr + v.y;
            }
            l = sl;
            r = sr;
            if (cnt > 1) {
                const float nf = (float)cnt;
                l = sl / nf;
                r = sr / nf;
            }
        }
        if constexpr (MONO) {
            float m = same && r > l ? r : l;
            if (!a.first) m = m > ox ? m : ox;
            a.col[py] = make_float2(m, m);
            if (have_b && !same) peak_update(b.col, py, b.first, r, r);
        } else {
            if (!a.first) {
                l = l > ox ? l : ox;
                r = r > oy ? r : oy;
            }
            a.col[py] = make_float2(l, r);
            oy = oy1; oy1 = oy2; oy2 = oy3;
        }
        ox = ox1; ox1 = ox2; ox2 = ox3;
        asm volatile("" ::: "memory");
    }
}

template <bool DUP>
__device__ __forceinline__ void store_row_f16(char *mags, long long row_byte, int col, const float (&va)[8], const float (&vb)[8], bool present = true)
{
    const __amdgpu_buffer_rsrc_t r = row_rsrc(mags, row_byte, present);
    const int lane_off = col * 4;
    const int lane_off0 = col != 0 ? lane_off : (int)0x80000000;
#pragma unroll
    for (int q3 = 0; q3 < 8; ++q3) {
        const __half2 h = __floats2half2_rn(va[q3], DUP ? va[q3] : vb[q3]);
        __builtin_amdgcn_raw_buffer_store_b32(*reinterpret_cast<const uint32_t *>(&h), r, (q3 == 0 ? lane_off0 : lane_off) + 1024 * (q3 & 3), 4096 * (q3 >> 2), 0);
    }
}

}
}
```

spectrogram_rs_amd/engine.py:

```python
from __future__ import annotations

import ctypes as C
from typing import Optional

import numpy as np

from . import _lib
from ._lib import SgxError, sgx_config, sgx_info


class SpectrogramEngine:
    def __init__(self, sample_rate: float = 48000.0, *, period: float = 0.0, stride: float = 0.0,
                 window_samples: int = 0, hop_samples: int = 0, channels: int = 1, rows: int = 1024,
                 f_min: float = 32.0, f_max: float = 22030.0, min_db: float = -70.0, max_db: float = -10.0,
                 interp: int = _lib.INTERP_CUBIC, lut_index_mode: int = _lib.LUT_FLOOR_N,
                 device: Optional[int] = None, force_generic: bool = False, gradient: Optional[str] = None,
                 fused_render: bool = True, lut_walk: bool = False,
                 mixed_generic: bool = False, complex_mono: bool = False, paired_frames: bool = False,
                 large_transforms: bool = False):
        import torch

        self._lib = _lib.load()
        self._ctx = C.c_void_p()
        cfg = sgx_config()
        self._lib.sgx_config_init(C.byref(cfg))
        cfg.sample_rate = sample_rate
        cfg.period, cfg.stride = period, stride
        if period == 0.0 and window_samples == 0:
            window_samples = 2048
        if stride == 0.0 and hop_samples == 0:
            hop_samples = 256
        cfg.window_samples, cfg.hop_samples = window_samples, hop_samples
        cfg.channels, cfg.rows = channels, rows
        cfg.f_min, cfg.f_max = f_min, f_max
        cfg.min_db, cfg.max_db = min_db, max_db
        cfg.interp, cfg.lut_index_mode = interp, lut_index_mode
        cfg.device = -1 if device is None else int(device)
        cfg.flags = (_lib.FLAG_FORCE_GENERIC if force_generic else 0) | (0 if fused_render else _lib.FLAG_NO_FUSED_RENDER) \
            | (_lib.FLAG_LUT_WALK if lut_walk else 0) | (_lib.FLAG_MIXED_GENERIC if mixed_generic else 0) \
            | (_lib.FLAG_COMPLEX_MONO if complex_mono else 0) | (_lib.FLAG_PAIRED_FRAMES if paired_frames else 0) \
            | (_lib.FLAG_LARGE_TRANSFORM if large_transforms else 0)
        if device is not None and torch.cuda.is_available():
            torch.cuda.set_device(int(device))
        rc = self._lib.sgx_create(C.byref(cfg), C.byref(self._ctx))
        if rc != 0:
            msg = self._lib.sgx_last_error(None).decode()
            self._ctx = C.c_void_p()
            raise SgxError(rc, msg)
        info = self._query()
        self.W, self.P, self.M, self.H = info.window_samples, info.fft_length, info.num_frequencies, info.hop_samples
        self.channels, self.pairs, self.R = info.channels, info.pairs, info.rows
        self.sample_rate = float(sample_rate)
        self.sample_rate_u32 = info.sample_rate_u32
        self.device = torch.device("cuda", torch.cuda.current_device() if device is None else int(device))
        self.use_current_stream()
        if gradient is not None:
            self.set_builtin_gradient(gradient)

    def _query(self):
        info = sgx_info()
        self._check(self._lib.sgx_query(self._ctx, C.byref(info)))
        self.info = info
        return info

    def _check(self, rc: int) -> int:
        if rc < 0:
            raise SgxError(rc, self._lib.sgx_last_error(self._ctx).decode())
        return rc

    def close(self):
        if getattr(self, "_ctx", None) is not None and self._ctx.value:
            for ref in list(getattr(self, "_rings", ())):
                ring = ref()
                if ring is not None:
                    ring.close()
            self._rings = []
            self._lib.sgx_destroy(self._ctx)
            self._ctx = C.c_void_p()

    def __del__(self):
        try:
            self.close()
        except Exception:
            pass

    def use_current_stream(self):
        import torch

        s = torch.cuda.current_stream(self.device)
        self._check(self._lib.sgx_set_stream(self._ctx, C.c_void_p(s.cuda_stream)))

    def set_stream(self, cuda_stream: int):
        self._check(self._lib.sgx_set_stream(self._ctx, C.c_void_p(cuda_stream)))

    def sync(self):
        self._check(self._lib.sgx_sync(self._ctx))

    def set_cu_limit(self, n: int):
        self._check(self._lib.sgx_set_cu_limit(self._ctx, C.c_uint32(n)))

    @property
    def cu_limit(self) -> int:
        return int(self._lib.sgx_cu_limit(self._ctx))

    def _dev_f32(self, t):
        import torch

        assert isinstance(t, torch.Tensor) and t.is_cuda and t.dtype == torch.float32 and t.is_contiguous(), \
            "expected a contiguous float32 CUDA tensor"
        assert t.device == self.device, f"tensor on {t.device}, engine on {self.device}"
        return C.c_void_p(t.data_ptr())

    def _out(self, out, shape, dtype):
        import torch

        self.use_current_stream()
        if out is None:
            return torch.empty(shape, dtype=dtype, device=self.device)
        need = 1
        for d in shape:
            need *= int(d)
        assert isinstance(out, torch.Tensor) and out.is_cuda and out.device == self.device, \
            f"out must be a CUDA tensor on {self.device}"
        assert out.dtype == dtype, f"out must be {dtype}, got {out.dtype}"
        assert out.is_contiguous(), "out must be contiguous"
        assert out.numel() >= need, f"out holds {out.numel()} elements, the call writes {need}"
        return out

    def num_frames(self, n_samples: int) -> int:
        return int(self._lib.sgx_num_frames(self._ctx, n_samples))

    def stft_batch(self, pcm, first_frame: int = 0, max_frames: Optional[int] = None, out=None):
        import torch

        n_samples = pcm.numel() // self.channels
        total = self.num_frames(n_samples)
        n = max(total - first_frame, 0)
        if max_frames is not None:
            n = min(n, max_frames)
        out = self._out(out, (n, self.pairs, self.M, 2), torch.float32)
        got = C.c_size_t(0)
        if n:
            self._check(self._lib.sgx_stft_batch(self._ctx, self._dev_f32(pcm), n_samples, first_frame, n,
                                                 C.c_void_p(out.data_ptr()), C.byref(got)))
            assert got.value == n
        return out

    def stft_batch_f16(self, pcm, first_frame: int = 0, max_frames: Optional[int] = None, out=None):
        import torch

        n_samples = pcm.numel() // self.channels
        total = self.num_frames(n_samples)
        n = max(total - first_frame, 0)
        if max_frames is not None:
            n = min(n, max_frames)
        out = self._out(out, (n, self.pairs, self.M, 2), torch.float16)
        got = C.c_size_t(0)
        if n:
            self._check(self._lib.sgx_stft_batch_f16(self._ctx, self._dev_f32(pcm), n_samples, first_frame, n,
                                                     C.c_void_p(out.data_ptr()), C.byref(got)))
            assert got.value == n
        return out

    def stft_batch_complex(self, pcm, first_frame: int = 0, max_frames: Optional[int] = None, out=None):
        import torch

        n_samples = pcm.numel() // self.channels
        total = self.num_frames(n_samples)
        n = max(total - first_frame, 0)
        if max_frames is not None:
            n = min(n, max_frames)
        if out is not None and out.dtype == torch.float32:
            buf = self._out(out, (n, self.pairs, self.M, 2, 2), torch.float32)
        else:
            buf = torch.view_as_real(self._out(out, (n, self.pairs, self.M, 2), torch.complex64))
        got = C.c_size_t(0)
        if n:
            self._check(self._lib.sgx_stft_batch_complex(self._ctx, self._dev_f32(pcm), n_samples, first_frame, n,
                                                         C.c_void_p(buf.data_ptr()), C.byref(got)))
            assert got.value == n
        return torch.view_as_complex(buf.reshape(-1)[:n * self.pairs * self.M * 4].view(n, self.pairs, self.M, 2, 2))

    def istft_batch(self, spec, first_sample: int = 0, max_samples: Optional[int] = None, out=None):
        import torch

        if spec.dtype == torch.complex64:
            spec = torch.view_as_real(spec)
        per_frame = self.pairs * self.M * 4
        assert spec.dtype == torch.float32 and spec.numel() % per_frame == 0, \
            "expected complex64 [frames][pairs][M][2] or float32 [frames][pairs][M][2][2]"
        n_frames = spec.numel() // per_frame
        total = (n_frames - 1) * self.H + self.W if n_frames else 0
        n = max(total - first_sample, 0)
        if max_samples is not None:
            n = min(n, max_samples)
        buf = self._out(out, (n, self.channels), torch.float32)
        got = C.c_size_t(0)
        self._check(self._lib.sgx_istft_batch(self._ctx, self._dev_f32(spec.contiguous()), n_frames, first_sample, n,
                                              C.c_void_p(buf.data_ptr()), C.byref(got)))
        assert got.value == n
        return buf.reshape(-1)[:n * self.channels].view(n, self.channels)

    def istft_supported(self) -> int:
        return self._check(self._lib.sgx_istft_supported(self._ctx))

    def process_one(self, lr: np.ndarray) -> Optional[np.ndarray]:
        lr = np.ascontiguousarray(lr, np.float32).reshape(-1, 2)
        out = np.empty((self.M, 2), np.float32)
        rc = self._check(self._lib.sgx_process_one(self._ctx, lr.ctypes.data_as(C.c_void_p), lr.shape[0],
                                                   out.ctypes.data_as(C.c_void_p)))
        return out if rc == 1 else None

    def render_batch(self, pcm, first_frame: int = 0, max_frames: Optional[int] = None, out=None):
        import torch

        n_samples = pcm.numel() // self.channels
        total = self.num_frames(n_samples)
        n = max(total - first_frame, 0)
        if max_frames is not None:
            n = min(n, max_frames)
        out = self._out(out, (n, self.pairs, self.R, 4), torch.uint8)
        got = C.c_size_t(0)
        if n:
            self._check(self._lib.sgx_render_batch(self._ctx, self._dev_f32(pcm), n_samples, first_frame, n,
                                                   C.c_void_p(out.data_ptr()), C.byref(got)))
            assert got.value == n
        return out

    def bands_batch(self, pcm, first_frame: int = 0, max_frames: Optional[int] = None, out=None):
        import torch

        n_samples = pcm.numel() // self.channels
        total = self.num_frames(n_samples)
        n = max(total - first_frame, 0)
        if max_frames is not None:
            n = min(n, max_frames)
        out = self._out(out, (n, self.pairs, self.R, 2), torch.float32)
        got = C.c_size_t(0)
        if n:
            self._check(self._lib.sgx_bands_batch(self._ctx, self._dev_f32(pcm), n_samples, first_frame, n,
                                                  C.c_void_p(out.data_ptr()), C.byref(got)))
            assert got.value == n
        return out

    @property
    def bands_fused(self) -> int:
        return self._check(self._lib.sgx_bands_fused(self._ctx))

    def bands_peak_batch(self, pcm, group: int, first_frame: int = 0, max_frames: Optional[int] = None, out=None):
        import torch

        n_samples = pcm.numel() // self.channels
        total = self.num_frames(n_samples)
        n = max(total - first_frame, 0)
        if max_frames is not None:
            n = min(n, max_frames)
        group = int(group)
        cols = -(-n // group) if group > 0 else 0
        out = self._out(out, (cols, self.pairs, self.R, 2), torch.float32)
        got = C.c_size_t(0)
        if n:
            self._check(self._lib.sgx_bands_peak_batch(self._ctx, self._dev_f32(pcm), n_samples, first_frame, n,
                                                       min(group, 2 ** 64 - 1), C.c_void_p(out.data_ptr()), C.byref(got)))
            assert got.value == cols
        return out

    @property
    def bands_peak_fused(self) -> int:
        return self._check(self._lib.sgx_bands_peak_fused(self._ctx))

    def _welch_batch(self, fn, comps, pcm, group, first_frame, max_frames, out):
        import torch

        n_samples = pcm.numel() // self.channels
        total = self.num_frames(n_samples)
        n = max(total - first_frame, 0)
        if max_frames is not None:
            n = min(n, max_frames)
        group = int(group)
        cols = -(-n // group) if group > 0 else 0
        out = self._out(out, (cols, self.pairs, self.M, comps), torch.float32)
        got = C.c_size_t(0)
        if n:
            self._check(fn(self._ctx, self._dev_f32(pcm), n_samples, first_frame, n, min(group, 2 ** 64 - 1),
                           C.c_void_p(out.data_ptr()), C.byref(got)))
            assert got.value == cols
        return out

    def _welch_rows(self, fn, comps, rows, row_floats, group, out):
        import torch

        assert rows.dtype == torch.float32 and rows.numel() % row_floats == 0, "expected whole float32 rows of this context"
        n = rows.numel() // row_floats
        group = int(group)
        cols = -(-n // group) if group > 0 else 0
        out = self._out(out, (cols, self.pairs, self.M, comps), torch.float32)
        got = C.c_size_t(0)
        if n:
            self._check(fn(self._ctx, self._dev_f32(rows), n, min(group, 2 ** 64 - 1), C.c_void_p(out.data_ptr()), C.byref(got)))
            assert got.value == cols
        return out

    def psd_batch(self, pcm, group: int, first_frame: int = 0, max_frames: Optional[int] = None, out=None):
        return self._welch_batch(self._lib.sgx_psd_batch, 2, pcm, group, first_frame, max_frames, out)

    def csd_batch(self, pcm, group: int, first_frame: int = 0, max_frames: Optional[int] = None, out=None):
        return self._welch_batch(self._lib.sgx_csd_batch, 4, pcm, group, first_frame, max_frames, out)

    def psd_mags(self, mags, group: int, out=None):
        return self._welch_rows(self._lib.sgx_psd_mags, 2, mags, self.pairs * self.M * 2, group, out)

    def csd_spec(self, spec, group: int, out=None):
        import torch

        if spec.dtype == torch.complex64:
            spec = torch.view_as_real(spec)
        return self._welch_rows(self._lib.sgx_csd_spec, 4, spec.contiguous(), self.pairs * self.M * 4, group, out)

    @property
    def psd_fused(self) -> int:
        return self._check(self._lib.sgx_psd_fused(self._ctx))

    @property
    def csd_fused(self) -> int:
        return self._check(self._lib.sgx_csd_fused(self._ctx))

    def filterbank(self, first, count, weights, power: int = 2) -> "FilterBank":
        import weakref

        fb = FilterBank(self, first, count, weights, power)
        if not hasattr(self, "_rings"):
            self._rings = []
        self._rings = [r for r in self._rings if r() is not None] + [weakref.ref(fb)]
        return fb

    def mel_filterbank(self, n_mels: int = 128, f_min: float = 0.0, f_max: Optional[float] = None, scale: str = "htk",
                       norm: Optional[str] = None, power: int = 2) -> "FilterBank":
        first, count, weights = mel_weights(self.sample_rate, self.W, n_mels, f_min, f_max, scale, norm)
        return self.filterbank(first, count, weights, power)

    def render_bands(self, bands, out=None):
        import torch

        n = bands.numel() // (self.R * 2)
        out = self._out(out, (n, self.R, 4), torch.uint8)
        if n:
            self._check(self._lib.sgx_render_bands(self._ctx, self._dev_f32(bands), n, C.c_void_p(out.data_ptr())))
        return out

    def render_mags(self, mags, out=None):
        import torch

        n = mags.numel() // (self.M * 2)
        out = self._out(out, (n, self.R, 4), torch.uint8)
        if n:
            self._check(self._lib.sgx_render_mags(self._ctx, self._dev_f32(mags), n, C.c_void_p(out.data_ptr())))
        return out

    def magnitude_in(self, mags, ranges: np.ndarray, out=None):
        import torch

        ranges = np.ascontiguousarray(ranges, np.float32).reshape(-1, 2)
        n = mags.numel() // (self.M * 2)
        out = self._out(out, (n, ranges.shape[0], 2), torch.float32)
        if n and ranges.shape[0]:
            self._check(self._lib.sgx_magnitude_in(self._ctx, self._dev_f32(mags), n, ranges.ctypes.data_as(C.c_void_p),
                                                   ranges.shape[0], C.c_void_p(out.data_ptr())))
        return out

    def spectrum_levels(self, column, levels: np.ndarray) -> np.ndarray:
        assert levels.dtype == np.float64 and levels.flags.c_contiguous
        assert column.numel() == self.M * 2
        self._check(self._lib.sgx_spectrum_levels(self._ctx, self._dev_f32(column), levels.size,
                                                  levels.ctypes.data_as(C.c_void_p)))
        return levels

    def live(self, capacity: int = 4096, reference_skip: bool = False) -> "LiveRing":
        import weakref

        ring = LiveRing(self, capacity, reference_skip)
        if not hasattr(self, "_rings"):
            self._rings = []
        self._rings = [r for r in self._rings if r() is not None] + [weakref.ref(ring)]
        return ring

    def image(self, width: int = 1024) -> "ImageRing":
        return ImageRing(self, width)

    def view(self, viewport_frames: int = 2048) -> "ViewRing":
        import weakref

        v = ViewRing(self, viewport_frames)
        if not hasattr(self, "_rings"):
            self._rings = []
        self._rings = [r for r in self._rings if r() is not None] + [weakref.ref(v)]
        return v

    def set_gradient(self, rgb: np.ndarray, stereo: bool = False):
        rgb = np.ascontiguousarray(rgb, np.uint8).reshape(-1, 3)
        self._check(self._lib.sgx_set_gradient(self._ctx, rgb.ctypes.data_as(C.c_void_p), rgb.shape[0], int(stereo)))
        self._query()

    def set_gradient_fn(self, fn, stereo: bool = False):
        def thunk(t, out, _user):
            r, g, b = fn(t)
            out[0], out[1], out[2] = int(r), int(g), int(b)
        self._gradient_cb = _lib.GRADIENT_FN(thunk)
        self._check(self._lib.sgx_set_gradient_fn(self._ctx, C.cast(self._gradient_cb, C.c_void_p), None, int(stereo)))
        self._query()

    def set_builtin_scheme(self, name: str, stereo: bool = False):
        self._check(self._lib.sgx_set_builtin_scheme(self._ctx, name.encode(), int(stereo)))
        self._query()

    def set_builtin_gradient(self, name: str):
        self._check(self._lib.sgx_set_builtin_gradient(self._ctx, name.encode()))
        self._query()

    def lookup_table(self, resolution: int = 32) -> np.ndarray:
        out = np.empty((resolution, resolution, 4), np.float32)
        self._check(self._lib.sgx_lookup_table(self._ctx, resolution, out.ctypes.data_as(C.c_void_p)))
        return out

    def bin_edges(self) -> np.ndarray:
        out = np.empty(self.R + 1, np.float32)
        self._check(self._lib.sgx_bin_edges(self._ctx, out.ctypes.data_as(C.c_void_p)))
        return out

    def row_sample_counts(self) -> np.ndarray:
        out = np.empty(self.R, np.uint32)
        self._check(self._lib.sgx_row_sample_counts(self._ctx, out.ctypes.data_as(C.c_void_p)))
        return out

    def window(self) -> np.ndarray:
        out = np.empty(self.W, np.float32)
        self._check(self._lib.sgx_window(self._ctx, out.ctypes.data_as(C.c_void_p)))
        return out

    def white_noise(self, n_samples: int, first: int = 0, seed: int = 0x5EED0001, channels: Optional[int] = None, out=None):
        import torch

        ch = self.channels if channels is None else channels
        out = self._out(out, (n_samples * ch,), torch.float32)
        self._check(self._lib.sgx_synth_white_noise(self._ctx, C.c_void_p(out.data_ptr()), first, n_samples, ch, seed))
        return out

    def checksum_add(self, t, acc, base_word: int = 0) -> None:
        import torch

        assert acc.is_cuda and acc.device == self.device and acc.dtype == torch.int64 and acc.numel() == 1
        assert t.is_cuda and t.device == self.device and t.is_contiguous()
        self.use_current_stream()
        self._check(self._lib.sgx_checksum_add(self._ctx, C.c_void_p(t.data_ptr()), t.numel() * t.element_size(),
                                               base_word, C.c_void_p(acc.data_ptr())))

    def checksum(self, t, base_word: int = 0) -> int:
        nbytes = t.numel() * t.element_size()
        v = C.c_uint64(0)
        self._check(self._lib.sgx_checksum(self._ctx, C.c_void_p(t.data_ptr()), nbytes, base_word, C.byref(v)))
        return int(v.value)


class LiveRing:

    _FORMATS = {"mags": (_lib.LIVE_MAGS, np.float32), "mags_f16": (_lib.LIVE_MAGS_F16, np.float16),
                "rgba": (_lib.LIVE_RGBA, np.uint8), "bands": (_lib.LIVE_BANDS, np.float32)}

    def __init__(self, engine: SpectrogramEngine, capacity: int = 4096, reference_skip: bool = False):
        self.engine = engine
        self.capacity = int(capacity)
        self._lib = engine._lib
        self._h = C.c_void_p()
        engine._check(self._lib.sgx_live_create(engine._ctx, self.capacity,
                                                _lib.LIVE_REFERENCE_SKIP if reference_skip else 0, C.byref(self._h)))

    def close(self):
        if getattr(self, "_h", None) is not None and self._h.value:
            self._lib.sgx_live_destroy(self._h)
            self._h = C.c_void_p()

    def __del__(self):
        try:
            self.close()
        except Exception:
            pass

    def push(self, data, channels: int) -> int:
        data = np.ascontiguousarray(data, np.float32).reshape(-1)
        n = int(self._lib.sgx_live_push(self._h, data.ctypes.data_as(C.c_void_p), data.size, channels))
        if n < 0:
            raise SgxError(n, f"{channels}-channel input not supported!" if n == _lib.SGX_ERR_UNSUPPORTED else "sgx_live_push")
        return n

    def occupied_len(self) -> int:
        return int(self._lib.sgx_live_occupied(self._h))

    def __len__(self) -> int:
        return self.occupied_len()

    def tick(self, what: str = "mags", max_frames: Optional[int] = None) -> np.ndarray:
        code, dtype = self._FORMATS[what]
        e = self.engine
        if max_frames is None:
            max_frames = e.num_frames(self.capacity)
        shape = {"rgba": (max_frames, e.R, 4), "bands": (max_frames, e.R, 2)}.get(what, (max_frames, e.M, 2))
        out = np.empty(shape, dtype)
        got = C.c_size_t(0)
        e._check(self._lib.sgx_live_tick(self._h, code, out.ctypes.data_as(C.c_void_p), max_frames, C.byref(got)))
        return out[:got.value]

    def tick_image(self, image: "ImageRing", max_frames: Optional[int] = None) -> int:
        e = self.engine
        if max_frames is None:
            max_frames = e.num_frames(self.capacity)
        e.use_current_stream()
        got = C.c_size_t(0)
        e._check(self._lib.sgx_live_tick_image(self._h, image._h, max_frames, C.byref(got)))
        return int(got.value)

    def tick_into(self, view: "ViewRing", max_frames: Optional[int] = None) -> int:
        e = self.engine
        if max_frames is None:
            max_frames = e.num_frames(self.capacity)
        got = C.c_size_t(0)
        e._check(self._lib.sgx_live_tick_view(self._h, view._h, max_frames, C.byref(got)))
        return int(got.value)


class FilterBank:

    def __init__(self, engine: SpectrogramEngine, first, count, weights, power: int = 2):
        self.engine = engine
        self._lib = engine._lib
        self._h = C.c_void_p()
        first = np.ascontiguousarray(first, np.uint32).reshape(-1)
        count = np.ascontiguousarray(count, np.uint32).reshape(-1)
        weights = np.ascontiguousarray(weights, np.float32).reshape(-1)
        assert first.size == count.size, "first and count hold one entry per filter"
        assert weights.size == int(count.sum(dtype=np.uint64)), "weights holds sum(count) entries"
        if weights.size == 0:
            weights = np.zeros(1, np.float32)
        engine.use_current_stream()
        engine._check(self._lib.sgx_fbank_create(engine._ctx, first.size, first.ctypes.data_as(C.c_void_p), count.ctypes.data_as(C.c_void_p),
                                                 weights.ctypes.data_as(C.c_void_p), int(power), C.byref(self._h)))
        self.power = int(power)
        self._n_weights = int(count.sum(dtype=np.uint64))

    def close(self):
        if getattr(self, "_h", None) is not None and self._h.value:
            self._lib.sgx_fbank_destroy(self._h)
            self._h = C.c_void_p()

    def __del__(self):
        try:
            self.close()
        except Exception:
            pass

    @property
    def n_filters(self) -> int:
        return int(self._lib.sgx_fbank_filters(self._h))

    @property
    def fused(self) -> int:
        return self.engine._check(self._lib.sgx_fbank_fused(self._h))

    def batch(self, pcm, first_frame: int = 0, max_frames: Optional[int] = None, out=None):
        import torch

        e = self.engine
        n_samples = pcm.numel() // e.channels
        total = e.num_frames(n_samples)
        n = max(total - first_frame, 0)
        if max_frames is not None:
            n = min(n, max_frames)
        out = e._out(out, (n, e.pairs, self.n_filters, 2), torch.float32)
        got = C.c_size_t(0)
        if n:
            e._check(self._lib.sgx_fbank_batch(self._h, e._dev_f32(pcm), n_samples, first_frame, n, C.c_void_p(out.data_ptr()), C.byref(got)))
            assert got.value == n
        return out

    def apply(self, mags, out=None):
        import torch

        e = self.engine
        n = mags.numel() // (e.M * 2)
        out = e._out(out, (n, self.n_filters, 2), torch.float32)
        if n:
            e._check(self._lib.sgx_fbank_mags(self._h, e._dev_f32(mags), n, C.c_void_p(out.data_ptr())))
        return out

    @property
    def cross_fused(self) -> int:
        return self.engine._check(self._lib.sgx_fbank_cross_fused(self._h))

    def cross_batch(self, pcm, first_frame: int = 0, max_frames: Optional[int] = None, out=None):
        import torch

        e = self.engine
        n_samples = pcm.numel() // e.channels
        total = e.num_frames(n_samples)
        n = max(total - first_frame, 0)
        if max_frames is not None:
            n = min(n, max_frames)
        out = e._out(out, (n, e.pairs, self.n_filters, 4), torch.float32)
        got = C.c_size_t(0)
        if n:
            e._check(self._lib.sgx_fbank_cross_batch(self._h, e._dev_f32(pcm), n_samples, first_frame, n, C.c_void_p(out.data_ptr()), C.byref(got)))
            assert got.value == n
        return out

    def cross_apply(self, spec, out=None):
        import torch

        e = self.engine
        if spec.dtype == torch.complex64:
            spec = torch.view_as_real(spec)
        n = spec.numel() // (e.M * 4)
        out = e._out(out, (n, self.n_filters, 4), torch.float32)
        if n:
            e._check(self._lib.sgx_fbank_cross_spec(self._h, e._dev_f32(spec), n, C.c_void_p(out.data_ptr())))
        return out


class ImageRing:

    def __init__(self, engine: SpectrogramEngine, width: int = 1024):
        self.engine = engine
        self.width, self.height = int(width), engine.R
        self._lib = engine._lib
        self._h = C.c_void_p()
        engine._check(self._lib.sgx_image_create(engine._ctx, self.width, C.byref(self._h)))

    def close(self):
        if getattr(self, "_h", None) is not None and self._h.value:
            self._lib.sgx_image_destroy(self._h)
            self._h = C.c_void_p()

    def __del__(self):
        try:
            self.close()
        except Exception:
            pass

    @property
    def offset(self) -> int:
        return int(self._lib.sgx_image_offset(self._h))

    def write_columns(self, rgba) -> int:
        import torch

        e = self.engine
        assert rgba.is_cuda and rgba.device == e.device and rgba.dtype == torch.uint8 and rgba.is_contiguous()
        n = rgba.numel() // (e.R * 4)
        assert rgba.numel() == n * e.R * 4
        e.use_current_stream()
        off = C.c_uint32(0)
        e._check(self._lib.sgx_image_write_columns(self._h, C.c_void_p(rgba.data_ptr()), n, C.byref(off)))
        return int(off.value)

    def read(self, scrolled: bool = False, out=None):
        import torch

        e = self.engine
        out = e._out(out, (self.height, self.width, 4), torch.uint8)
        e._check(self._lib.sgx_image_read(self._h, 1 if scrolled else 0, C.c_void_p(out.data_ptr())))
        return out


class ViewRing:

    def __init__(self, engine: SpectrogramEngine, viewport_frames: int = 2048):
        self.engine = engine
        self.rows = int(viewport_frames)
        self._lib = engine._lib
        self._h = C.c_void_p()
        engine._check(self._lib.sgx_view_create(engine._ctx, self.rows, C.byref(self._h)))

    def close(self):
        if getattr(self, "_h", None) is not None and self._h.value:
            self._lib.sgx_view_destroy(self._h)
            self._h = C.c_void_p()

    def __del__(self):
        try:
            self.close()
        except Exception:
            pass

    @property
    def offset(self) -> int:
        return int(self._lib.sgx_view_offset(self._h))

    def write_rows(self, rows_f16) -> int:
        import torch

        e = self.engine
        assert rows_f16.is_cuda and rows_f16.device == e.device and rows_f16.dtype == torch.float16 and rows_f16.is_contiguous()
        n = rows_f16.numel() // (e.M * 2)
        assert rows_f16.numel() == n * e.M * 2
        e.use_current_stream()
        off = C.c_uint32(0)
        e._check(self._lib.sgx_view_write_rows(self._h, C.c_void_p(rows_f16.data_ptr()), n, C.byref(off)))
        return int(off.value)

    def draw(self, width: int, height: int, out=None):
        import torch

        e = self.engine
        out = e._out(out, (height, width, 4), torch.float32)
        e._check(self._lib.sgx_view_draw(self._h, width, height, C.c_void_p(out.data_ptr())))
        return out


def builtin_gradient_eval(name: str, t: float):
    lib = _lib.load()
    out = (C.c_uint8 * 3)()
    if lib.sgx_builtin_gradient_eval(name.encode(), float(t), out) != 0:
        raise KeyError(name)
    return tuple(int(x) for x in out)


def builtin_gradient(name: str) -> np.ndarray:
    lib = _lib.load()
    out = np.empty((256, 3), np.uint8)
    if lib.sgx_builtin_gradient(name.encode(), out.ctypes.data_as(C.c_void_p)) != 0:
        raise KeyError(name)
    return out


_MEL_SCALES = {"htk": _lib.MEL_HTK, "slaney": _lib.MEL_SLANEY}
_MEL_NORMS = {None: _lib.MEL_NORM_NONE, "none": _lib.MEL_NORM_NONE, "slaney": _lib.MEL_NORM_SLANEY}


def mel_weights(sample_rate: float, window_samples: int, n_mels: int = 128, f_min: float = 0.0, f_max: Optional[float] = None,
                scale: str = "htk", norm: Optional[str] = None):
    lib = _lib.load()
    if f_max is None:
        f_max = sample_rate / 2.0
    args = (C.c_double(sample_rate), int(window_samples), int(n_mels), C.c_double(f_min), C.c_double(f_max), _MEL_SCALES[scale], _MEL_NORMS[norm])
    n = C.c_size_t(0)
    rc = lib.sgx_mel_weights(*args, None, None, None, C.byref(n))
    if rc != 0:
        raise SgxError(rc, "sgx_mel_weights: invalid argument")
    first, count = np.zeros(n_mels, np.uint32), np.zeros(n_mels, np.uint32)
    weights = np.zeros(max(n.value, 1), np.float32)
    rc = lib.sgx_mel_weights(*args, first.ctypes.data_as(C.c_void_p), count.ctypes.data_as(C.c_void_p), weights.ctypes.data_as(C.c_void_p), C.byref(n))
    if rc != 0:
        raise SgxError(rc, "sgx_mel_weights: invalid argument")
    return first, count, weights[:n.value]
```

Measured before the change: 304.5 million.

## Add hybrid static/atomic-claimed job scheduling to the real 4096 STFT kernel

Blocks in the non-fused real 4096-point STFT kernel now take a static share of jobs, by default twelve sixteenths of the total. After that they claim chunks of the remaining jobs through a global atomic counter, which is meant to reduce the tail imbalance across blocks. It adds a per-launch memset, an atomic per claimed chunk, a small amount of LDS, and Params fields that share unions with the render fields. An API to set and query the split is exposed, along with debug timestamps for block finish times.

```diff
diff --git a/bindings/rust/sgx_sys.rs b/bindings/rust/sgx_sys.rs
--- a/bindings/rust/sgx_sys.rs
+++ b/bindings/rust/sgx_sys.rs
@@ -72,6 +72,8 @@
     pub fn sgx_sync(ctx: *mut SgxCtx) -> c_int;
     pub fn sgx_set_cu_limit(ctx: *mut SgxCtx, n: u32) -> c_int;
     pub fn sgx_cu_limit(ctx: *const SgxCtx) -> u32;
+    pub fn sgx_set_run_claim(ctx: *mut SgxCtx, static_sixteenths: u32, chunk_jobs: u32) -> c_int;
+    pub fn sgx_run_claim(ctx: *const SgxCtx, n_frames: usize, static_sixteenths: *mut u32, chunk_jobs: *mut u32) -> c_int;
 }
 extern "C" {
     pub fn hipMalloc(p: *mut *mut c_void, bytes: usize) -> c_int;
diff --git a/include/sgx.h b/include/sgx.h
--- a/include/sgx.h
+++ b/include/sgx.h
@@ -93,6 +93,9 @@
 SGX_API int sgx_set_cu_limit(sgx_ctx *ctx, uint32_t n);
 SGX_API uint32_t sgx_cu_limit(const sgx_ctx *ctx);
 
+SGX_API int sgx_set_run_claim(sgx_ctx *ctx, uint32_t static_sixteenths, uint32_t chunk_jobs);
+SGX_API int sgx_run_claim(const sgx_ctx *ctx, size_t n_frames, uint32_t *static_sixteenths, uint32_t *chunk_jobs);
+
 
 SGX_API int sgx_stft_batch(sgx_ctx *ctx, const float *d_pcm, size_t n_samples, size_t first_frame,
                            size_t max_frames, float *d_mags, size_t *n_out);
diff --git a/spectrogram_rs_amd/_lib.py b/spectrogram_rs_amd/_lib.py
--- a/spectrogram_rs_amd/_lib.py
+++ b/spectrogram_rs_amd/_lib.py
@@ -88,6 +88,8 @@
     ("sgx_sync", C.c_int, [_ctx]),
     ("sgx_set_cu_limit", C.c_int, [_ctx, C.c_uint32]),
     ("sgx_cu_limit", C.c_uint32, [_ctx]),
+    ("sgx_set_run_claim", C.c_int, [_ctx, C.c_uint32, C.c_uint32]),
+    ("sgx_run_claim", C.c_int, [_ctx, _sz, C.POINTER(C.c_uint32), C.POINTER(C.c_uint32)]),
     ("sgx_stft_batch", C.c_int, [_ctx, _vp, _sz, _sz, _sz, _vp, C.POINTER(_sz)]),
     ("sgx_stft_batch_f16", C.c_int, [_ctx, _vp, _sz, _sz, _sz, _vp, C.POINTER(_sz)]),
     ("sgx_stft_batch_complex", C.c_int, [_ctx, _vp, _sz, _sz, _sz, _vp, C.POINTER(_sz)]),
diff --git a/spectrogram_rs_amd/csrc/run_claim.hpp b/spectrogram_rs_amd/csrc/run_claim.hpp
--- /dev/null
+++ b/spectrogram_rs_amd/csrc/run_claim.hpp
@@ -0,0 +1,42 @@
+#pragma once
+
+namespace sgx {
+
+struct RunClaim {
+    unsigned long long per;
+    unsigned long long pool_begin;
+    unsigned long long n_chunks;
+    unsigned long long chunk;
+};
+struct JobRun { unsigned long long begin, end; };
+
+inline RunClaim run_claim(unsigned long long n_jobs, unsigned long long blocks, unsigned static_sixteenths, unsigned long long chunk_jobs)
+{
+    RunClaim r;
+    r.per = (n_jobs / 16 * static_sixteenths + n_jobs % 16 * static_sixteenths / 16) / blocks;
+    r.pool_begin = blocks * r.per;
+    r.chunk = chunk_jobs < 1 ? 1 : chunk_jobs;
+    r.n_chunks = (n_jobs - r.pool_begin + r.chunk - 1) / r.chunk;
+    return r;
+}
+inline JobRun static_run(const RunClaim &r, unsigned long long block) { return {block * r.per, (block + 1) * r.per}; }
+inline JobRun claimed_run(const RunClaim &r, unsigned long long n_jobs, unsigned long long i)
+{
+    if (i >= r.n_chunks) return {n_jobs, n_jobs};
+    const unsigned long long b = r.pool_begin + i * r.chunk, left = n_jobs - b;
+    return {b, b + (left < r.chunk ? left : r.chunk)};
+}
+
+constexpr unsigned kClaimAutoSixteenths = 12, kClaimAutoChunk = 8;
+constexpr unsigned long long kClaimMinStatic = 64;
+inline bool run_claim_engages(unsigned long long n_jobs, unsigned long long blocks)
+{
+    return run_claim(n_jobs, blocks, kClaimAutoSixteenths, kClaimAutoChunk).per >= kClaimMinStatic;
+}
+inline bool run_claim_valid(unsigned static_sixteenths, unsigned chunk_jobs)
+{
+    if (chunk_jobs == 0) return static_sixteenths == 0 || static_sixteenths == 16;
+    return static_sixteenths <= 16 && chunk_jobs <= (1u << 20);
+}
+
+}
diff --git a/spectrogram_rs_amd/csrc/sgx_internal.hpp b/spectrogram_rs_amd/csrc/sgx_internal.hpp
--- a/spectrogram_rs_amd/csrc/sgx_internal.hpp
+++ b/spectrogram_rs_amd/csrc/sgx_internal.hpp
@@ -152,6 +152,7 @@
 
     int n_cu = 256;
     int n_cu_device = 256;
+    uint32_t claim_sixteenths = 0, claim_chunk = 0;
     size_t lds_optin = 64 * 1024;
     mutable std::vector<std::pair<std::array<size_t, 3>, int>> occupancy_cache;
     std::vector<struct sgx_view *> views;
diff --git a/spectrogram_rs_amd/csrc/stft4096_real.hip b/spectrogram_rs_amd/csrc/stft4096_real.hip
--- a/spectrogram_rs_amd/csrc/stft4096_real.hip
+++ b/spectrogram_rs_amd/csrc/stft4096_real.hip
@@ -1,6 +1,7 @@
 #include <cmath>
 #include <type_traits>
 
+#include "run_claim.hpp"
 #include "stft4096_wg.hpp"
 
 namespace sgx {
@@ -98,6 +99,12 @@
 
 #if SGX_STAMPS
 __device__ unsigned long long g_phase_cycles_r[24];
+constexpr int kFinishBlocks = 4096;
+__device__ unsigned long long g_finish_r[4 * kFinishBlocks];
+#if SGX_STAMPS == 2
+#undef SGX_STAMP
+#define SGX_STAMP(i)
+#endif
 #endif
 
 template <int MODE, int PIX, bool SLIDE>
@@ -113,6 +120,9 @@
     constexpr bool FUSED = MODE == kPixels || MODE == kBands || MODE == kPeak || MODE == kFbank;
 
     const int tid = threadIdx.x;
+#if SGX_STAMPS
+    if (tid == 0 && blockIdx.x < kFinishBlocks) g_finish_r[4 * blockIdx.x] = wall_clock64();
+#endif
     const int t_p1 = TR ? (tid >> 4) + 16 * (tid & 15) : tid;
     float *plane = reinterpret_cast<float *>(smem_raw);
     const uint32_t m0_wave = __builtin_amdgcn_readfirstlane((uint32_t)(tid >> 6) * 272u);
@@ -144,13 +154,20 @@
     const int cbase2 = (g2 >> 3) * 128 + (g2 & 7);
     __syncthreads();
 
-    const unsigned long long job_begin = (unsigned long long)blockIdx.x * p.jobs_per_block;
+#ifdef SGX_VARIANT_SKIP_LAST_JOB
+    constexpr bool CLAIM = false;
+#else
+    constexpr bool CLAIM = !FUSED;
+#endif
+    const bool claiming = CLAIM && p.claim_counter != nullptr;
+    unsigned long long *claim_word = reinterpret_cast<unsigned long long *>(tw2 + 256);
+    unsigned long long job_begin = (unsigned long long)blockIdx.x * p.jobs_per_block;
     unsigned long long job_end = job_begin + p.jobs_per_block;
     if (job_end > p.n_jobs) job_end = p.n_jobs;
 #ifdef SGX_VARIANT_SKIP_LAST_JOB
     if (job_end > job_begin + 1) --job_end;
 #endif
-    if (job_begin >= job_end) return;
+    if (job_begin >= job_end && !claiming) return;
 
     auto samples_from = [&](unsigned long long first) {
         const unsigned long long left = first < p.stream_samples ? (p.stream_samples - first) * 4 : 0;
@@ -171,287 +188,315 @@
 #pragma unroll
         for (int a = 0; a < 4; ++a) { R[2 * a] = column(r0, 2048 * a); R[2 * a + 1] = column(r1, 2048 * a); }
     };
-    {
-        const __amdgpu_buffer_rsrc_t r0 = columns_from(128 * (p.first_frame + 2 * job_begin));
-        if (SLIDE) {
-#pragma unroll
-            for (int j = 0; j < 8; ++j) R[j] = column(r0, 1024 * j);
-            L = column(r0, 9216);
-        } else {
-            load_pair(p.first_frame + 2 * job_begin);
-            L = R[7];
-        }
-#pragma unroll
-        for (int j = 0; j < 8; ++j) asm volatile("" ::"v"(R[j].x), "v"(R[j].y));
-        asm volatile("" ::"v"(L.x), "v"(L.y));
-#pragma unroll
-        for (int q = 1; q < 8; ++q) asm volatile("" ::"v"(tw1[q].x), "v"(tw1[q].y));
-#pragma unroll
-        for (int q = 0; q < 8; ++q) asm volatile("" ::"v"(twu[q].x), "v"(twu[q].y), "v"(win[q]));
-    }
     float2 *xch = buf + 2304;
-
     char *out = reinterpret_cast<char *>(p.mags);
     constexpr int kBin = C64 ? 16 : (F16 ? 4 : 8);
 #if SGX_STAMPS
     unsigned long long st_acc[20] = {0, 0, 0, 0, 0, 0, 0, 0, 0, 0, 0, 0, 0, 0, 0, 0, 0, 0, 0, 0};
     unsigned long long st_last = __builtin_readcyclecounter();
-#endif
-    for (unsigned long long job = job_begin; job < job_end; ++job) {
-        SGX_STAMP(19)
-        const unsigned long long fa = p.first_frame + 2 * job;
-        const unsigned long long la = 2 * job, lb = la + 1;
-        const bool have_b = lb < p.n_frames;
-
-        float yr[8], yi[8];
+    unsigned long long jobs_done = 0;
+#endif
+    for (;;) {
         {
-            float zr[4], zi[4];
-#pragma unroll
-            for (int a = 0; a < 4; ++a) { zr[a] = R[2 * a].x * win[2 * a]; zi[a] = R[2 * a].y * win[2 * a + 1]; }
-            fft8_half_zero(zr, zi, yr, yi);
+            const __amdgpu_buffer_rsrc_t r0 = columns_from(128 * (p.first_frame + 2 * job_begin));
+            if (SLIDE) {
+#pragma unroll
+                for (int j = 0; j < 8; ++j) R[j] = column(r0, 1024 * j);
+                L = column(r0, 9216);
+            } else {
+                load_pair(p.first_frame + 2 * job_begin);
+                L = R[7];
+            }
+            if (claiming && tid == 0) {
+                unsigned long long claimed;
+                asm volatile("global_atomic_add_x2 %0, %1, %2, off sc0\n\t"
+                             "s_waitcnt vmcnt(0)"
+                             : "=&v"(claimed)
+                             : "v"(p.claim_counter), "v"(1ull)
+                             : "memory");
+                *claim_word = claimed;
+            }
+#pragma unroll
+            for (int j = 0; j < 8; ++j) asm volatile("" ::"v"(R[j].x), "v"(R[j].y));
+            asm volatile("" ::"v"(L.x), "v"(L.y));
+#pragma unroll
+            for (int q = 1; q < 8; ++q) asm volatile("" ::"v"(tw1[q].x), "v"(tw1[q].y));
+#pragma unroll
+            for (int q = 0; q < 8; ++q) asm volatile("" ::"v"(twu[q].x), "v"(twu[q].y), "v"(win[q]));
         }
-        float vr[8], vi[8];
-        {
-            float zr[4], zi[4];
-#pragma unroll
-            for (int a = 0; a < 4; ++a) { zr[a] = R[2 * a + 1].x * win[2 * a]; zi[a] = R[2 * a + 1].y * win[2 * a + 1]; }
-            fft8_half_zero(zr, zi, vr, vi);
+        for (unsigned long long job = job_begin; job < job_end; ++job) {
+            SGX_STAMP(19)
+            const unsigned long long fa = p.first_frame + 2 * job;
+            const unsigned long long la = 2 * job, lb = la + 1;
+            const bool have_b = lb < p.n_frames;
+
+            float yr[8], yi[8];
+            {
+                float zr[4], zi[4];
+#pragma unroll
+                for (int a = 0; a < 4; ++a) { zr[a] = R[2 * a].x * win[2 * a]; zi[a] = R[2 * a].y * win[2 * a + 1]; }
+                fft8_half_zero(zr, zi, yr, yi);
+            }
+            float vr[8], vi[8];
+            {
+                float zr[4], zi[4];
+#pragma unroll
+                for (int a = 0; a < 4; ++a) { zr[a] = R[2 * a + 1].x * win[2 * a]; zi[a] = R[2 * a + 1].y * win[2 * a + 1]; }
+                fft8_half_zero(zr, zi, vr, vi);
+            }
+            SGX_STAMP(0)
+            lds_barrier();
+            SGX_STAMP(1)
+#pragma unroll
+            for (int q = 0; q < 8; ++q) {
+                const float2 ya = make_float2(yr[q], yi[q]), yb = make_float2(vr[q], vi[q]);
+                if (TR) {
+                    addtid_rows<272>(q == 0 ? ya : cmulf(ya, tw1[q]), q == 0 ? yb : cmulf(yb, tw1[q]), m0_wave, q, 8 + q);
+                } else {
+                    buf[q * kS1 + tid] = q == 0 ? ya : cmulf(ya, tw1[q]);
+                    buf[(8 + q) * kS1 + tid] = q == 0 ? yb : cmulf(yb, tw1[q]);
+                }
+            }
+            __builtin_amdgcn_s_setprio(0);
+            SGX_STAMP(2)
+            lds_barrier();
+            SGX_STAMP(3)
+
+            float xr[16], xi[16];
+            if (TR) {
+                read_planes(rd4_1, xr, xi);
+            } else {
+#pragma unroll
+                for (int t1 = 0; t1 < 16; ++t1) {
+                    const float2 v = buf[g2 * kS1 + t0_2 + 16 * t1];
+                    xr[t1] = v.x; xi[t1] = v.y;
+                }
+            }
+            fft16(xr, xi);
+            SGX_STAMP(4)
+            lds_barrier();
+            SGX_STAMP(5)
+            if (TR) {
+                lds_cfloat2 *tw2p = lds_ptr(tw2 + t0_2);
+#pragma unroll
+                for (int q2 = 0; q2 < 16; q2 += 2) {
+                    const int pa = FFT16_OUT[q2], pb = FFT16_OUT[q2 + 1];
+                    const float2 va = make_float2(xr[pa], xi[pa]), vb = make_float2(xr[pb], xi[pb]);
+                    addtid_rows<280>(q2 == 0 ? va : cmulf(va, lds_read_alone(tw2p, q2 * 16)), cmulf(vb, lds_read_alone(tw2p, (q2 + 1) * 16)), m0_wave, q2, q2 + 1);
+                }
+            } else {
+#pragma unroll
+                for (int q2 = 0; q2 < 16; ++q2) {
+                    const int pos = FFT16_OUT[q2];
+                    const float2 v = make_float2(xr[pos], xi[pos]);
+                    buf[t0_2 * kS2 + cbase2 + 8 * q2] = q2 == 0 ? v : cmulf(v, tw2[q2 * 16 + t0_2]);
+                }
+            }
+            SGX_STAMP(6)
+            lds_barrier();
+            SGX_STAMP(7)
+
+            if (TR) {
+                read_planes(rd4_2, xr, xi);
+            } else {
+#pragma unroll
+                for (int t0 = 0; t0 < 16; ++t0) {
+                    const float2 v = buf[t0 * kS2 + tid];
+                    xr[t0] = v.x; xi[t0] = v.y;
+                }
+            }
+            fft16(xr, xi);
+
+            float2 Ln = make_float2(0.0f, 0.0f);
+            if (SLIDE && !FUSED) Ln = column(columns_from(128 * (fa + 2) + 1152), 0);
+            if (!SLIDE) load_pair(fa + 2);
+
+            if (FUSED) __builtin_amdgcn_s_setprio(1);
+            else __builtin_amdgcn_s_setprio(3);
+            SGX_STAMP(8)
+            lds_barrier();
+            SGX_STAMP(9)
+#pragma unroll
+            for (int j = 0; j < 8; ++j) {
+                const int pos = FFT16_OUT[8 + j];
+                buf[j * 256 + tid] = make_float2(xr[pos], xi[pos]);
+            }
+            if (SLIDE && !TR) {
+                xch[tid].x = tid < 128 ? L.x : R[7].x;
+                xch[tid].y = tid < 128 ? L.y : R[7].y;
+            }
+            SGX_STAMP(10)
+            lds_barrier();
+            SGX_STAMP(11)
+            if (SLIDE) {
+                const float2 Y = TR ? make_float2(lane_xor8((tid & 8) ? R[7].x : L.x), lane_xor8((tid & 8) ? R[7].y : L.y)) : xch[(tid + 128) & 255];
+#pragma unroll
+                for (int j = 0; j < 6; ++j) R[j] = R[j + 2];
+                R[6] = Y;
+                R[7] = L;
+            }
+
+            const int pcol = F * 128 + (u == 0 ? 256 : 128 - u);
+            float m1[8], m2[8];
+            constexpr bool kInterleave = (!FUSED && SLIDE) || C64;
+            const long long row = (long long)(F == 0 ? la : lb) * (long long)kM * kBin - kBin;
+            const __amdgpu_buffer_rsrc_t r = out_rsrc(out, !FUSED ? row : 0, !FUSED && (F == 0 || have_b));
+            const int l1 = kBin * u, l2 = kBin * (1152 - u);
+            auto store_pair = [&](const int q3) {
+                const float a = m1[q3], b = (q3 == 0 && u == 0) ? m1[0] : m2[q3];
+                const int o1 = (q3 == 0 && u == 0) ? kBin * 1024 : l1;
+                const int o2 = (q3 == 0 && u == 0) ? kBin * 128 : l2;
+                const int s1 = kBin * 128 * q3, s2 = kBin * 128 * (7 - q3);
+                if (F16) {
+                    const __half2 ha = __floats2half2_rn(a, a), hb = __floats2half2_rn(b, b);
+                    __builtin_amdgcn_raw_buffer_store_b32(*reinterpret_cast<const uint32_t *>(&ha), r, o1 + (s1 & 2047), s1 & ~2047, 0);
+                    __builtin_amdgcn_raw_buffer_store_b32(*reinterpret_cast<const uint32_t *>(&hb), r, o2 + (s2 & 2047), s2 & ~2047, 0);
+                } else {
+                    __builtin_amdgcn_raw_buffer_store_b64(u32x2{__float_as_uint(a), __float_as_uint(a)}, r, o1 + (s1 & 2047), s1 & ~2047, 0);
+                    __builtin_amdgcn_raw_buffer_store_b64(u32x2{__float_as_uint(b), __float_as_uint(b)}, r, o2 + (s2 & 2047), s2 & ~2047, 0);
+                }
+            };
+            float2 pvs[8];
+            if (kInterleave) {
+#pragma unroll
+                for (int q3 = 0; q3 < 8; ++q3) pvs[q3] = buf[(7 - q3) * 256 + pcol];
+            }
+#pragma unroll
+            for (int q3 = 0; q3 < 8; ++q3) {
+                const int pos = FFT16_OUT[q3];
+                float zr_ = xr[pos], zi_ = xi[pos];
+                float2 pv = kInterleave ? pvs[q3] : buf[(7 - q3) * 256 + pcol];
+                if (q3 == 0) {
+                    const float2 own = buf[F * 128];
+                    const int p8 = FFT16_OUT[8];
+                    zr_ = u == 0 ? xr[p8] : zr_; zi_ = u == 0 ? xi[p8] : zi_;
+                    pv.x = u == 0 ? own.x : pv.x; pv.y = u == 0 ? own.y : pv.y;
+                }
+                const float er = zr_ + pv.x, ei = zi_ - pv.y;
+                const float orr = zi_ + pv.y, oi = pv.x - zr_;
+                const float wr = fmaf(twu[q3].x, orr, -(twu[q3].y * oi)), wi = fmaf(twu[q3].x, oi, twu[q3].y * orr);
+                const float ar = er + wr, ai = ei + wi, br = er - wr, bi = ei - wi;
+                if constexpr (C64) {
+                    const bool self = q3 == 0 && u == 0;
+                    const float cr2 = self ? ar : br, ci2 = self ? ai : -bi;
+                    const int o1 = self ? kBin * 1024 : l1, o2 = self ? kBin * 128 : l2;
+                    const int s1 = kBin * 128 * q3, s2 = kBin * 128 * (7 - q3);
+                    __builtin_amdgcn_raw_buffer_store_b128(u32x4{__float_as_uint(ar), __float_as_uint(ai), __float_as_uint(ar), __float_as_uint(ai)}, r, o1 + s1, 0, 0);
+                    __builtin_amdgcn_raw_buffer_store_b128(u32x4{__float_as_uint(cr2), __float_as_uint(ci2), __float_as_uint(cr2), __float_as_uint(ci2)}, r, o2 + s2, 0, 0);
+                    __builtin_amdgcn_sched_barrier(0);
+                    continue;
+                }
+                m1[q3] = __builtin_amdgcn_sqrtf(fmaf(ar, ar, ai * ai));
+                m2[q3] = __builtin_amdgcn_sqrtf(fmaf(br, br, bi * bi));
+                if (kInterleave) {
+                    store_pair(q3);
+                    __builtin_amdgcn_sched_barrier(0);
+                }
+            }
+
+            if (!FUSED) {
+                if (!kInterleave) {
+#pragma unroll
+                    for (int q3 = 0; q3 < 8; ++q3) store_pair(q3);
+                }
+            } else {
+                float2 *mpair = buf;
+                float2 *vbuf = mpair + wg::kColSlots;
+                float *mcol = reinterpret_cast<float *>(buf) + F;
+                lds_barrier();
+                SGX_STAMP(13)
+                constexpr bool kEarlyWords = PIX != wg::kPixGeneric && MODE != kFbank;
+                wg::SampleWords sw;
+                const __amdgpu_buffer_rsrc_t rt_words = wg::pcm_rsrc(reinterpret_cast<const float *>(p.samples));
+                int tid_w = tid;
+                asm volatile("" : "+v"(tid_w));
+#pragma unroll
+                for (int q3 = 0; q3 < 8; ++q3) {
+                    const bool self = q3 == 0 && u == 0;
+                    const int k1 = self ? 1024 : u + 128 * q3, k2 = self ? 1024 : 2048 - u - 128 * q3;
+                    mcol[2 * k1] = m1[q3];
+                    mcol[2 * k2] = self ? m1[0] : m2[q3];
+                    if (q3 == 0 && u == 1) {
+                        mcol[0] = m1[0];
+                        mcol[2 * (kM + 1)] = mcol[2 * (kM + 2)] = m2[0];
+                    }
+                    if (kEarlyWords) {
+                        sw.se[q3] = wg::sample_word(rt_words, p, (uint32_t)tid_w + 256u * q3);
+                        __builtin_amdgcn_sched_barrier(0);
+                    }
+                }
+                if (kEarlyWords) sw.se[8] = wg::sample_word(rt_words, p, (uint32_t)tid_w + 2048u);
+                static_assert(wg::kSampleSteps == 9 && wg::kSampleEarly == 9, "one word per column-write step and one behind them");
+                SGX_STAMP(14)
+                lds_barrier();
+                SGX_STAMP(15)
+                if constexpr (MODE == kFbank) {
+                    float2 *sums = reinterpret_cast<float2 *>(p.rgba);
+                    __builtin_amdgcn_s_setprio(3);
+                    fbank::filter_pass<true>(mpair + 1, reinterpret_cast<const fbank::Filter *>(p.rows), reinterpret_cast<const float *>(p.samples), p.R,
+                                             p.interp == 2u, sums + la * (size_t)p.R, sums + lb * (size_t)p.R, true, have_b, (uint32_t)tid, 4u);
+                    if (SLIDE) L = column(columns_from(128 * (fa + 2) + 1152), 0);
+                } else {
+                if (kEarlyWords) wg::sample_pass_with<PIX>(p, mpair, vbuf, tid, sw);
+                else wg::sample_pass<PIX>(p, mpair, vbuf, tid);
+                [[maybe_unused]] wg::PeakDst peak_a{}, peak_b{};
+                [[maybe_unused]] wg::PeakOld<true> peak_old{};
+                if constexpr (MODE == kPeak) {
+                    peak_a = wg::peak_dst(p, la);
+                    peak_b = have_b ? wg::peak_dst_next(p, peak_a, lb) : peak_a;
+                    peak_old = wg::peak_prefetch<true>(p, peak_a, tid);
+                }
+                if (SLIDE) L = column(columns_from(128 * (fa + 2) + 1152), 0);
+                SGX_STAMP(16)
+                lds_barrier();
+                SGX_STAMP(17)
+                __builtin_amdgcn_s_setprio(3);
+                if constexpr (MODE == kPeak) {
+                    wg::row_pass_peak<true>(p, row_words, vbuf, peak_a, peak_b, peak_old, have_b, tid);
+                } else if constexpr (MODE == kBands) {
+                    float2 *bands = reinterpret_cast<float2 *>(p.rgba);
+                    wg::row_pass_bands<true>(p, row_words, vbuf, bands + la * (size_t)p.R, bands + lb * (size_t)p.R, true, have_b, tid);
+                } else {
+                    uchar4 *rgba = reinterpret_cast<uchar4 *>(p.rgba);
+                    wg::row_pass<true, PIX>(p, row_words, vbuf, rgba + la * (size_t)p.R, rgba + lb * (size_t)p.R, true, have_b, pal, tid);
+                }
+                }
+            }
+            if (SLIDE && !FUSED) {
+                asm volatile("" : "+v"(Ln.x), "+v"(Ln.y));
+                L = Ln;
+            }
+            SGX_STAMP(18)
         }
-        SGX_STAMP(0)
+#if SGX_STAMPS
+        jobs_done += job_end - job_begin;
+#endif
+        if (!claiming) break;
         lds_barrier();
-        SGX_STAMP(1)
-#pragma unroll
-        for (int q = 0; q < 8; ++q) {
-            const float2 ya = make_float2(yr[q], yi[q]), yb = make_float2(vr[q], vi[q]);
-            if (TR) {
-                addtid_rows<272>(q == 0 ? ya : cmulf(ya, tw1[q]), q == 0 ? yb : cmulf(yb, tw1[q]), m0_wave, q, 8 + q);
-            } else {
-                buf[q * kS1 + tid] = q == 0 ? ya : cmulf(ya, tw1[q]);
-                buf[(8 + q) * kS1 + tid] = q == 0 ? yb : cmulf(yb, tw1[q]);
-            }
-        }
-        __builtin_amdgcn_s_setprio(0);
-        SGX_STAMP(2)
+        const unsigned long long word = *claim_word;
+        const unsigned long long chunk_i = ((unsigned long long)__builtin_amdgcn_readfirstlane((uint32_t)(word >> 32)) << 32) | __builtin_amdgcn_readfirstlane((uint32_t)word);
         lds_barrier();
-        SGX_STAMP(3)
-
-        float xr[16], xi[16];
-        if (TR) {
-            read_planes(rd4_1, xr, xi);
-        } else {
-#pragma unroll
-            for (int t1 = 0; t1 < 16; ++t1) {
-                const float2 v = buf[g2 * kS1 + t0_2 + 16 * t1];
-                xr[t1] = v.x; xi[t1] = v.y;
-            }
-        }
-        fft16(xr, xi);
-        SGX_STAMP(4)
-        lds_barrier();
-        SGX_STAMP(5)
-        if (TR) {
-            lds_cfloat2 *tw2p = lds_ptr(tw2 + t0_2);
-#pragma unroll
-            for (int q2 = 0; q2 < 16; q2 += 2) {
-                const int pa = FFT16_OUT[q2], pb = FFT16_OUT[q2 + 1];
-                const float2 va = make_float2(xr[pa], xi[pa]), vb = make_float2(xr[pb], xi[pb]);
-                addtid_rows<280>(q2 == 0 ? va : cmulf(va, lds_read_alone(tw2p, q2 * 16)), cmulf(vb, lds_read_alone(tw2p, (q2 + 1) * 16)), m0_wave, q2, q2 + 1);
-            }
-        } else {
-#pragma unroll
-            for (int q2 = 0; q2 < 16; ++q2) {
-                const int pos = FFT16_OUT[q2];
-                const float2 v = make_float2(xr[pos], xi[pos]);
-                buf[t0_2 * kS2 + cbase2 + 8 * q2] = q2 == 0 ? v : cmulf(v, tw2[q2 * 16 + t0_2]);
-            }
-        }
-        SGX_STAMP(6)
-        lds_barrier();
-        SGX_STAMP(7)
-
-        if (TR) {
-            read_planes(rd4_2, xr, xi);
-        } else {
-#pragma unroll
-            for (int t0 = 0; t0 < 16; ++t0) {
-                const float2 v = buf[t0 * kS2 + tid];
-                xr[t0] = v.x; xi[t0] = v.y;
-            }
-        }
-        fft16(xr, xi);
-
-        float2 Ln = make_float2(0.0f, 0.0f);
-        if (SLIDE && !FUSED) Ln = column(columns_from(128 * (fa + 2) + 1152), 0);
-        if (!SLIDE) load_pair(fa + 2);
-
-        if (FUSED) __builtin_amdgcn_s_setprio(1);
-        else __builtin_amdgcn_s_setprio(3);
-        SGX_STAMP(8)
-        lds_barrier();
-        SGX_STAMP(9)
-#pragma unroll
-        for (int j = 0; j < 8; ++j) {
-            const int pos = FFT16_OUT[8 + j];
-            buf[j * 256 + tid] = make_float2(xr[pos], xi[pos]);
-        }
-        if (SLIDE && !TR) {
-            xch[tid].x = tid < 128 ? L.x : R[7].x;
-            xch[tid].y = tid < 128 ? L.y : R[7].y;
-        }
-        SGX_STAMP(10)
-        lds_barrier();
-        SGX_STAMP(11)
-        if (SLIDE) {
-            const float2 Y = TR ? make_float2(lane_xor8((tid & 8) ? R[7].x : L.x), lane_xor8((tid & 8) ? R[7].y : L.y)) : xch[(tid + 128) & 255];
-#pragma unroll
-            for (int j = 0; j < 6; ++j) R[j] = R[j + 2];
-            R[6] = Y;
-            R[7] = L;
-        }
-
-        const int pcol = F * 128 + (u == 0 ? 256 : 128 - u);
-        float m1[8], m2[8];
-        constexpr bool kInterleave = (!FUSED && SLIDE) || C64;
-        const long long row = (long long)(F == 0 ? la : lb) * (long long)kM * kBin - kBin;
-        const __amdgpu_buffer_rsrc_t r = out_rsrc(out, !FUSED ? row : 0, !FUSED && (F == 0 || have_b));
-        const int l1 = kBin * u, l2 = kBin * (1152 - u);
-        auto store_pair = [&](const int q3) {
-            const float a = m1[q3], b = (q3 == 0 && u == 0) ? m1[0] : m2[q3];
-            const int o1 = (q3 == 0 && u == 0) ? kBin * 1024 : l1;
-            const int o2 = (q3 == 0 && u == 0) ? kBin * 128 : l2;
-            const int s1 = kBin * 128 * q3, s2 = kBin * 128 * (7 - q3);
-            if (F16) {
-                const __half2 ha = __floats2half2_rn(a, a), hb = __floats2half2_rn(b, b);
-                __builtin_amdgcn_raw_buffer_store_b32(*reinterpret_cast<const uint32_t *>(&ha), r, o1 + (s1 & 2047), s1 & ~2047, 0);
-                __builtin_amdgcn_raw_buffer_store_b32(*reinterpret_cast<const uint32_t *>(&hb), r, o2 + (s2 & 2047), s2 & ~2047, 0);
-            } else {
-                __builtin_amdgcn_raw_buffer_store_b64(u32x2{__float_as_uint(a), __float_as_uint(a)}, r, o1 + (s1 & 2047), s1 & ~2047, 0);
-                __builtin_amdgcn_raw_buffer_store_b64(u32x2{__float_as_uint(b), __float_as_uint(b)}, r, o2 + (s2 & 2047), s2 & ~2047, 0);
-            }
-        };
-        float2 pvs[8];
-        if (kInterleave) {
-#pragma unroll
-            for (int q3 = 0; q3 < 8; ++q3) pvs[q3] = buf[(7 - q3) * 256 + pcol];
-        }
-#pragma unroll
-        for (int q3 = 0; q3 < 8; ++q3) {
-            const int pos = FFT16_OUT[q3];
-            float zr_ = xr[pos], zi_ = xi[pos];
-            float2 pv = kInterleave ? pvs[q3] : buf[(7 - q3) * 256 + pcol];
-            if (q3 == 0) {
-                const float2 own = buf[F * 128];
-                const int p8 = FFT16_OUT[8];
-                zr_ = u == 0 ? xr[p8] : zr_; zi_ = u == 0 ? xi[p8] : zi_;
-                pv.x = u == 0 ? own.x : pv.x; pv.y = u == 0 ? own.y : pv.y;
-            }
-            const float er = zr_ + pv.x, ei = zi_ - pv.y;
-            const float orr = zi_ + pv.y, oi = pv.x - zr_;
-            const float wr = fmaf(twu[q3].x, orr, -(twu[q3].y * oi)), wi = fmaf(twu[q3].x, oi, twu[q3].y * orr);
-            const float ar = er + wr, ai = ei + wi, br = er - wr, bi = ei - wi;
-            if constexpr (C64) {
-                const bool self = q3 == 0 && u == 0;
-                const float cr2 = self ? ar : br, ci2 = self ? ai : -bi;
-                const int o1 = self ? kBin * 1024 : l1, o2 = self ? kBin * 128 : l2;
-                const int s1 = kBin * 128 * q3, s2 = kBin * 128 * (7 - q3);
-                __builtin_amdgcn_raw_buffer_store_b128(u32x4{__float_as_uint(ar), __float_as_uint(ai), __float_as_uint(ar), __float_as_uint(ai)}, r, o1 + s1, 0, 0);
-                __builtin_amdgcn_raw_buffer_store_b128(u32x4{__float_as_uint(cr2), __float_as_uint(ci2), __float_as_uint(cr2), __float_as_uint(ci2)}, r, o2 + s2, 0, 0);
-                __builtin_amdgcn_sched_barrier(0);
-                continue;
-            }
-            m1[q3] = __builtin_amdgcn_sqrtf(fmaf(ar, ar, ai * ai));
-            m2[q3] = __builtin_amdgcn_sqrtf(fmaf(br, br, bi * bi));
-            if (kInterleave) {
-                store_pair(q3);
-                __builtin_amdgcn_sched_barrier(0);
-            }
-        }
-
-        if (!FUSED) {
-            if (!kInterleave) {
-#pragma unroll
-                for (int q3 = 0; q3 < 8; ++q3) store_pair(q3);
-            }
-        } else {
-            float2 *mpair = buf;
-            float2 *vbuf = mpair + wg::kColSlots;
-            float *mcol = reinterpret_cast<float *>(buf) + F;
-            lds_barrier();
-            SGX_STAMP(13)
-            constexpr bool kEarlyWords = PIX != wg::kPixGeneric && MODE != kFbank;
-            wg::SampleWords sw;
-            const __amdgpu_buffer_rsrc_t rt_words = wg::pcm_rsrc(reinterpret_cast<const float *>(p.samples));
-            int tid_w = tid;
-            asm volatile("" : "+v"(tid_w));
-#pragma unroll
-            for (int q3 = 0; q3 < 8; ++q3) {
-                const bool self = q3 == 0 && u == 0;
-                const int k1 = self ? 1024 : u + 128 * q3, k2 = self ? 1024 : 2048 - u - 128 * q3;
-                mcol[2 * k1] = m1[q3];
-                mcol[2 * k2] = self ? m1[0] : m2[q3];
-                if (q3 == 0 && u == 1) {
-                    mcol[0] = m1[0];
-                    mcol[2 * (kM + 1)] = mcol[2 * (kM + 2)] = m2[0];
-                }
-                if (kEarlyWords) {
-                    sw.se[q3] = wg::sample_word(rt_words, p, (uint32_t)tid_w + 256u * q3);
-                    __builtin_amdgcn_sched_barrier(0);
-                }
-            }
-            if (kEarlyWords) sw.se[8] = wg::sample_word(rt_words, p, (uint32_t)tid_w + 2048u);
-            static_assert(wg::kSampleSteps == 9 && wg::kSampleEarly == 9, "one word per column-write step and one behind them");
-            SGX_STAMP(14)
-            lds_barrier();
-            SGX_STAMP(15)
-            if constexpr (MODE == kFbank) {
-                float2 *sums = reinterpret_cast<float2 *>(p.rgba);
-                __builtin_amdgcn_s_setprio(3);
-                fbank::filter_pass<true>(mpair + 1, reinterpret_cast<const fbank::Filter *>(p.rows), reinterpret_cast<const float *>(p.samples), p.R,
-                                         p.interp == 2u, sums + la * (size_t)p.R, sums + lb * (size_t)p.R, true, have_b, (uint32_t)tid, 4u);
-                if (SLIDE) L = column(columns_from(128 * (fa + 2) + 1152), 0);
-            } else {
-            if (kEarlyWords) wg::sample_pass_with<PIX>(p, mpair, vbuf, tid, sw);
-            else wg::sample_pass<PIX>(p, mpair, vbuf, tid);
-            [[maybe_unused]] wg::PeakDst peak_a{}, peak_b{};
-            [[maybe_unused]] wg::PeakOld<true> peak_old{};
-            if constexpr (MODE == kPeak) {
-                peak_a = wg::peak_dst(p, la);
-                peak_b = have_b ? wg::peak_dst_next(p, peak_a, lb) : peak_a;
-                peak_old = wg::peak_prefetch<true>(p, peak_a, tid);
-            }
-            if (SLIDE) L = column(columns_from(128 * (fa + 2) + 1152), 0);
-            SGX_STAMP(16)
-            lds_barrier();
-            SGX_STAMP(17)
-            __builtin_amdgcn_s_setprio(3);
-            if constexpr (MODE == kPeak) {
-                wg::row_pass_peak<true>(p, row_words, vbuf, peak_a, peak_b, peak_old, have_b, tid);
-            } else if constexpr (MODE == kBands) {
-                float2 *bands = reinterpret_cast<float2 *>(p.rgba);
-                wg::row_pass_bands<true>(p, row_words, vbuf, bands + la * (size_t)p.R, bands + lb * (size_t)p.R, true, have_b, tid);
-            } else {
-                uchar4 *rgba = reinterpret_cast<uchar4 *>(p.rgba);
-                wg::row_pass<true, PIX>(p, row_words, vbuf, rgba + la * (size_t)p.R, rgba + lb * (size_t)p.R, true, have_b, pal, tid);
-            }
-            }
-        }
-        if (SLIDE && !FUSED) {
-            asm volatile("" : "+v"(Ln.x), "+v"(Ln.y));
-            L = Ln;
-        }
-        SGX_STAMP(18)
+        if (chunk_i >= p.claim_chunks) break;
+        job_begin = p.claim_pool_begin + chunk_i * p.claim_chunk;
+        job_end = job_begin + p.claim_chunk < p.n_jobs ? job_begin + p.claim_chunk : p.n_jobs;
     }
 #if SGX_STAMPS
+    if (tid == 0 && blockIdx.x < kFinishBlocks) {
+        g_finish_r[4 * blockIdx.x + 1] = wall_clock64();
+        g_finish_r[4 * blockIdx.x + 2] = blockIdx.x;
+        g_finish_r[4 * blockIdx.x + 3] = jobs_done;
+    }
     if ((tid & 63) == 0) {
 #pragma unroll
         for (int i = 0; i < 20; ++i) atomicAdd(&g_phase_cycles_r[i], st_acc[i]);
-        atomicAdd(&g_phase_cycles_r[20], (unsigned long long)(job_end - job_begin));
+        atomicAdd(&g_phase_cycles_r[20], jobs_done);
     }
 #endif
 }
 
 struct RealTables {
     DeviceBuffer<float2> d_tw1, d_tw2, d_twu;
+    DeviceBuffer<unsigned long long> d_claim;
 };
 
 }
@@ -465,6 +510,11 @@
         e = hipMemcpyToSymbol(HIP_SYMBOL(wgr::g_phase_cycles_r), zero, sizeof(zero));
     }
     return e == hipSuccess ? 0 : -1;
+}
+extern "C" __attribute__((visibility("default"))) int sgx_debug_finish_r(unsigned long long *h_out, int n_blocks)
+{
+    if (n_blocks < 0 || n_blocks > wgr::kFinishBlocks) return -1;
+    return hipMemcpyFromSymbol(h_out, HIP_SYMBOL(wgr::g_finish_r), sizeof(unsigned long long) * 4 * (size_t)n_blocks) == hipSuccess ? 0 : -1;
 }
 #endif
 
@@ -485,6 +535,7 @@
     hipError_t e = t->d_tw1.upload(tw1);
     if (e == hipSuccess) e = t->d_tw2.upload(tw2);
     if (e == hipSuccess) e = t->d_twu.upload(twu);
+    if (e == hipSuccess) e = t->d_claim.alloc(1);
     if (e == hipSuccess) c->real = std::move(t);
     return e;
 }
@@ -496,6 +547,21 @@
 }
 
 namespace wg {
+
+struct RowsClaim { uint32_t sixteenths, chunk; };
+static RowsClaim rows_claim(const sgx_ctx *c, Out kind, unsigned long long n_jobs, unsigned long long blocks)
+{
+    const bool rows = kind == Out::kMags || kind == Out::kMagsF16 || kind == Out::kComplex;
+#ifdef SGX_VARIANT_SKIP_LAST_JOB
+    const bool compiled = false;
+#else
+    const bool compiled = true;
+#endif
+    if (!rows || !compiled || n_jobs == 0 || (c->claim_sixteenths == 16u && c->claim_chunk == 0u)) return {16u, 0u};
+    if (c->claim_chunk != 0u) return {c->claim_sixteenths, c->claim_chunk};
+    if (kind == Out::kComplex) return {16u, 0u};
+    return run_claim_engages(n_jobs, blocks) ? RowsClaim{kClaimAutoSixteenths, kClaimAutoChunk} : RowsClaim{16u, 0u};
+}
 
 hipError_t launch_real4096(const sgx_ctx *c, Params p, Out kind)
 {
@@ -514,10 +580,23 @@
         p.peak_run = 2 * runs.per;
     }
     p.jobs_per_block = runs.per;
+    const RowsClaim rc = rows_claim(c, kind, p.n_jobs, runs.blocks);
+    if (rc.sixteenths != 16u || rc.chunk != 0u) {
+        const RunClaim split = run_claim(p.n_jobs, runs.blocks, rc.sixteenths, rc.chunk);
+        const hipError_t e = hipMemsetAsync(t->d_claim.get(), 0, sizeof(unsigned long long), c->stream);
+        if (e != hipSuccess) return e;
+        p.jobs_per_block = split.per;
+        p.claim_counter = t->d_claim.get();
+        p.claim_pool_begin = split.pool_begin;
+        p.claim_chunks = split.n_chunks;
+        p.claim_chunk = (uint32_t)split.chunk;
+    }
+    const size_t lds_claim = p.claim_counter ? sizeof(unsigned long long) : 0;
     const dim3 grid((unsigned)runs.blocks), block(256);
     auto launch = [&](auto slide_c) {
         constexpr bool S_ = decltype(slide_c)::value;
-        constexpr size_t lds_rows = S_ ? kLdsBytesR : kLdsBytes, lds_render = S_ ? kLdsBytesRenderR : kLdsBytesRender;
+        const size_t lds_rows = (S_ ? kLdsBytesR : kLdsBytes) + lds_claim;
+        constexpr size_t lds_render = S_ ? kLdsBytesRenderR : kLdsBytesRender;
         if (hold_peak) {
             if (p.interp == SGX_INTERP_COSINE) hipLaunchKernelGGL((stft4096_real_kernel<kPeak, kPixPeakCosine, S_>), grid, block, lds_rows, c->stream, p);
             else hipLaunchKernelGGL((stft4096_real_kernel<kPeak, kPixPeakCubic, S_>), grid, block, lds_rows, c->stream, p);
@@ -547,3 +626,28 @@
 }
 
 }
+
+int sgx_set_run_claim(sgx_ctx *c, uint32_t static_sixteenths, uint32_t chunk_jobs)
+{
+    if (!c) return SGX_ERR_INVALID_ARG;
+    if (!sgx::run_claim_valid(static_sixteenths, chunk_jobs)) {
+        c->err = "sgx_set_run_claim: a share of 0 .. 16 sixteenths with a chunk of 1 .. 2^20 jobs, (16, 0) for the static split or (0, 0) for the automatic rule";
+        return SGX_ERR_INVALID_ARG;
+    }
+    c->claim_sixteenths = static_sixteenths;
+    c->claim_chunk = chunk_jobs;
+    return SGX_OK;
+}
+
+int sgx_run_claim(const sgx_ctx *c, size_t n_frames, uint32_t *static_sixteenths, uint32_t *chunk_jobs)
+{
+    if (!c || !static_sixteenths || !chunk_jobs) return SGX_ERR_INVALID_ARG;
+    sgx::wg::RowsClaim rc{16u, 0u};
+    if (sgx::real4096_serves(c, nullptr, c->C) && !(c->cfg.flags & (SGX_FLAG_PAIRED_FRAMES | SGX_FLAG_COMPLEX_MONO))) {
+        const unsigned long long n_jobs = ((unsigned long long)n_frames + 1) / 2;
+        rc = sgx::wg::rows_claim(c, sgx::Out::kMags, n_jobs, sgx::run_split(c, n_jobs, 4).blocks);
+    }
+    *static_sixteenths = rc.sixteenths;
+    *chunk_jobs = rc.chunk;
+    return SGX_OK;
+}
diff --git a/spectrogram_rs_amd/csrc/stft4096_wg.hpp b/spectrogram_rs_amd/csrc/stft4096_wg.hpp
--- a/spectrogram_rs_amd/csrc/stft4096_wg.hpp
+++ b/spectrogram_rs_amd/csrc/stft4096_wg.hpp
@@ -34,9 +34,18 @@
     unsigned long long total_frames;
     uint32_t H, C, pair_l, pair_r, pairs, pair;
     uint32_t out_f16;
-    const uint32_t *rows;
-    const PackedSample *samples;
-    uint32_t n_samples;
+    union {
+        const uint32_t *rows;
+        unsigned long long *claim_counter;
+    };
+    union {
+        const PackedSample *samples;
+        unsigned long long claim_pool_begin;
+    };
+    union {
+        uint32_t n_samples;
+        uint32_t claim_chunk;
+    };
     union {
         const float *lut_thr;
         unsigned long long peak_group;
@@ -45,7 +54,10 @@
         const uchar4 *lut_rgba;
         unsigned long long peak_run;
     };
-    uint8_t *rgba;
+    union {
+        uint8_t *rgba;
+        unsigned long long claim_chunks;
+    };
     uint32_t R, interp;
     float guess_a, guess_b;
     uint32_t seed_pm1;
diff --git a/spectrogram_rs_amd/engine.py b/spectrogram_rs_amd/engine.py
--- a/spectrogram_rs_amd/engine.py
+++ b/spectrogram_rs_amd/engine.py
@@ -103,6 +103,14 @@
     def cu_limit(self) -> int:
         return int(self._lib.sgx_cu_limit(self._ctx))
 
+    def set_run_claim(self, static_sixteenths: int, chunk_jobs: int):
+        self._check(self._lib.sgx_set_run_claim(self._ctx, C.c_uint32(static_sixteenths), C.c_uint32(chunk_jobs)))
+
+    def run_claim(self, n_frames: int):
+        s, k = C.c_uint32(), C.c_uint32()
+        self._check(self._lib.sgx_run_claim(self._ctx, C.c_size_t(n_frames), C.byref(s), C.byref(k)))
+        return int(s.value), int(k.value)
+
     def _dev_f32(self, t):
         import torch
 
```

After: 312.5 million (median of 6 runs). +2.6%, better.
